# SerCharles/CN-RMA

Measured on AMD Instinct MI355X. Metric: scenes/sec fwd (40-view->192^3 voxel): dense unprojection + RMA + voxelise + FCAF3D + decode, higher is better.
Workload: dtype f32 (sparse conv f16x3: 22-bit operands, fp32 accumulate; value_f32_conv = exact fp32); 1 GPU; NS: 40 views x 256 ch x 480x640 fp32 maps (channels_last) -> grid 192x192x192, N=300, max_points=500000, FCAF3D MinkResNet34 + head, 1 HIP graph per scene, 3 in flight; M_rows=72216505, M_selected=500000, M_unique=496819

## Files before the change

### cn-rma_amd/csrc/dense.hip

```cpp
#include "common.h"


namespace {

static __device__ __forceinline__ int64_t ceil_div_dev(int64_t a, int64_t b) { return (a + b - 1) / b; }

struct DenseParams {
  int V, C, H, W, X, Y, Z;
  float vs, ox, oy, oz;
};

__device__ __forceinline__ void voxel_world(const DenseParams& p, int64_t g, float* wx, float* wy, float* wz) {
  const int z = (int)(g % p.Z);
  const int64_t t = g / p.Z;
  const int y = (int)(t % p.Y);
  const int x = (int)(t / p.Y);
  *wx = (float)x * p.vs + p.ox;
  *wy = (float)y * p.vs + p.oy;
  *wz = (float)z * p.vs + p.oz;
}

struct SlabOrder { int on, nsx, nsy, nsz, zt, st, tt, zi, nt, own, stagger, groups; };

__device__ __forceinline__ bool slab_decode(const DenseParams& p, const SlabOrder& o, int64_t gv, int* x, int* y, int* z) {
  const int64_t per = (int64_t)o.st * o.st * o.zt;
  const int64_t sv = gv / per;
  const int r = (int)(gv - sv * per);
  if (sv >= (int64_t)o.nsx * o.nsy * o.nsz) return false;
  const int sy = (int)(sv % o.nsy), sx = (int)((sv / o.nsy) % o.nsx), sz = (int)(sv / ((int64_t)o.nsy * o.nsx));
  const int tcols = o.tt * o.tt, zo_n = o.zt / o.zi;
  const int zin = r % o.zi, q = r / o.zi;
  const int in = q % tcols, q2 = q / tcols;
  const int zo = q2 % zo_n, tile = q2 / zo_n;
  const int zl = zo * o.zi + zin;
  const int tpr = o.st / o.tt;
  *x = sx * o.st + (tile / tpr) * o.tt + in / o.tt;
  *y = sy * o.st + (tile % tpr) * o.tt + in % o.tt;
  *z = sz * o.zt + zl;
  return *x < p.X && *y < p.Y && *z < p.Z;
}

__device__ __forceinline__ bool lattice_decode(const DenseParams& p, const SlabOrder& o, int64_t lb, int tid, int* x, int* y, int* z) {
  const int cb = o.st * o.st / 8;
  const int64_t sv = lb / cb;
  if (sv >= (int64_t)o.nsx * o.nsy * o.nsz) return false;
  const int w = (int)(lb - sv * cb), j = tid >> 5, q4 = o.st / 4;
  const int sy = (int)(sv % o.nsy), sx = (int)((sv / o.nsy) % o.nsx), sz = (int)(sv / ((int64_t)o.nsy * o.nsx));
  *x = sx * o.st + w / q4 + (o.st / 2) * (j >> 2);
  *y = sy * o.st + w % q4 + q4 * (j & 3);
  *z = sz * 32 + (tid & 31);
  return *x < p.X && *y < p.Y && *z < p.Z;
}

__device__ __forceinline__ bool project(const float* __restrict__ P, float wx, float wy, float wz, int H, int W,
                                        float* rx, float* ry) {
  float cam[3];
#pragma unroll
  for (int r = 0; r < 3; ++r) {
    float acc = P[r * 4 + 0] * wx;
    acc = fmaf(P[r * 4 + 1], wy, acc);
    acc = fmaf(P[r * 4 + 2], wz, acc);
    acc = fmaf(P[r * 4 + 3], 1.0f, acc);
    cam[r] = acc;
  }
  *rx = rintf(cam[0] / cam[2]);
  *ry = rintf(cam[1] / cam[2]);
  return (*rx >= 0.0f) && (*ry >= 0.0f) && (*rx < (float)W) && (*ry < (float)H) && (cam[2] > 0.0f);
}

template <int CT>
__global__ __launch_bounds__(256) void backproject_accum_kernel(DenseParams p, const float* __restrict__ feat,
                                                                const float* __restrict__ proj,
                                                                float* __restrict__ volume,
                                                                int32_t* __restrict__ count) {
  const int64_t G = (int64_t)p.X * p.Y * p.Z;
  const int64_t g = (int64_t)blockIdx.x * blockDim.x + threadIdx.x;
  if (g >= G) return;
  const int c0 = blockIdx.y * CT;
  float wx, wy, wz;
  voxel_world(p, g, &wx, &wy, &wz);
  float acc[CT];
#pragma unroll
  for (int c = 0; c < CT; ++c) acc[c] = 0.0f;
  int cnt = 0;
  const int64_t plane = (int64_t)p.H * p.W * p.C;
  for (int v = 0; v < p.V; ++v) {
    float rx, ry;
    if (!project(proj + v * 12, wx, wy, wz, p.H, p.W, &rx, &ry)) continue;
    ++cnt;
    const float* f = feat + v * plane + ((int64_t)(int)ry * p.W + (int)rx) * p.C + c0;
    if constexpr (CT % 4 == 0) {
#pragma unroll
      for (int c = 0; c < CT; c += 4) {
        float4 q = *reinterpret_cast<const float4*>(f + c);
        acc[c] += q.x; acc[c + 1] += q.y; acc[c + 2] += q.z; acc[c + 3] += q.w;
      }
    } else {
#pragma unroll
      for (int c = 0; c < CT; ++c) acc[c] += f[c];
    }
  }
  const float denom = (float)cnt;
#pragma unroll
  for (int c = 0; c < CT; ++c) {
    if (c0 + c < p.C) volume[(int64_t)(c0 + c) * G + g] = cnt > 0 ? acc[c] / denom : 0.0f;
  }
  if (blockIdx.y == 0) count[g] = cnt;
}

__device__ __forceinline__ void group_barrier(unsigned int* w, unsigned int n) {
  __syncthreads();
  if (threadIdx.x == 0) {
    const unsigned int old = __hip_atomic_fetch_add(w, 1u, __ATOMIC_RELAXED, __HIP_MEMORY_SCOPE_AGENT);
    const unsigned int goal = (old / n + 1u) * n;
    for (int spin = 0; spin < 1024; ++spin) {
      if ((int)(__hip_atomic_load(w, __ATOMIC_RELAXED, __HIP_MEMORY_SCOPE_AGENT) - goal) >= 0) break;
      __builtin_amdgcn_s_sleep(64);
    }
  }
  __syncthreads();
}

template <int LPV, int EPI>
__device__ __forceinline__ int group_src_lane(int grp, int vsel) {
  constexpr int VPG = 64 / LPV;
  if constexpr (EPI == 0 && LPV >= 4) return (grp / 4) * (4 * VPG) + vsel * 4 + (grp % 4);
  else return grp * VPG + vsel;
}

typedef float dense_f4 __attribute__((ext_vector_type(4)));

template <int ELEM> struct DenseElem { typedef float type; typedef float4 load_t; static constexpr int Q = 1; };
template <> struct DenseElem<CNRMA_ELEM_F16> { typedef uint16_t type; typedef uint4 load_t; static constexpr int Q = 2; };
template <> struct DenseElem<CNRMA_ELEM_BF16> { typedef uint16_t type; typedef uint4 load_t; static constexpr int Q = 2; };

__device__ __forceinline__ void store_run(float* o, float a, float b, float c, float d, int policy) {
  dense_f4 v = {a, b, c, d};
  if (policy == 1) __builtin_nontemporal_store(v, reinterpret_cast<dense_f4*>(o));
  else if (policy == 2) asm volatile("global_store_dwordx4 %0, %1, off sc1\n\ts_nop 1" : : "v"(o), "v"(v) : "memory");
  else *reinterpret_cast<dense_f4*>(o) = v;
}

template <int LPV, int PIPE, int EPI, int ELEM = 0>
__device__ __forceinline__ void accum_block(const DenseParams& p, const typename DenseElem<ELEM>::type* __restrict__ feat,
                                            const float* __restrict__ proj, float* __restrict__ volume,
                                            int32_t* __restrict__ count, int64_t lb, int c0, bool write_count,
                                            const SlabOrder& ord, float* __restrict__ lds_wave, int tid) {
  constexpr int VPG = 64 / LPV;
  constexpr int Q = DenseElem<ELEM>::Q, CPL = 4 * Q;
  typedef typename DenseElem<ELEM>::type feat_t;
  typedef typename DenseElem<ELEM>::load_t load_t;
  static_assert(EPI != 1 || ELEM == 0, "the LDS-transposed epilogue exists for fp32 maps only");
  const int64_t G = (int64_t)p.X * p.Y * p.Z;
  const int lane = tid & 63;
  const int64_t g = lb * 256 + tid;
  float wx = 0.f, wy = 0.f, wz = 0.f;
  bool in_grid;
  int64_t lin = -1;
  if (ord.on) {
    int x = 0, y = 0, z = 0;
    in_grid = ord.on == 2 ? lattice_decode(p, ord, lb, tid, &x, &y, &z) : slab_decode(p, ord, g, &x, &y, &z);
    if (in_grid) {
      lin = ((int64_t)x * p.Y + y) * p.Z + z;
      wx = (float)x * p.vs + p.ox; wy = (float)y * p.vs + p.oy; wz = (float)z * p.vs + p.oz;
    }
  } else {
    in_grid = g < G;
    if (in_grid) { voxel_world(p, g, &wx, &wy, &wz); lin = g; }
  }
  if (__ballot(in_grid) == 0ull) return;
  float4 acc[LPV * Q];
#pragma unroll
  for (int i = 0; i < LPV * Q; ++i) acc[i] = make_float4(0.f, 0.f, 0.f, 0.f);
  int cnt = 0;
  int sub = lane % LPV, vsel = lane / LPV;
  const int64_t plane = (int64_t)p.H * p.W * p.C;
  const feat_t* fbase = feat + c0 + CPL * sub;

  auto pixel_of = [&](int v) -> int {
    float rx, ry;
    const bool ok = in_grid && project(proj + v * 12, wx, wy, wz, p.H, p.W, &rx, &ry);
    return ok ? ((int)ry * p.W + (int)rx) : -1;
  };
  auto gather = [&](int v, int pix, load_t* q) {
    const feat_t* fv = fbase + v * plane;
#pragma unroll
    for (int grp = 0; grp < LPV; ++grp) {
      const int pq = __shfl(pix, group_src_lane<LPV, EPI>(grp, vsel), 64);
      if constexpr (ELEM == 0) q[grp] = make_float4(0.f, 0.f, 0.f, 0.f);
      else q[grp] = make_uint4(0u, 0u, 0u, 0u);
      if (pq >= 0) q[grp] = *reinterpret_cast<const load_t*>(fv + (int64_t)pq * p.C);
    }
  };
  auto add = [&](const load_t* q) {
#pragma unroll
    for (int grp = 0; grp < LPV; ++grp) {
      if constexpr (ELEM == 0) {
        acc[grp].x += q[grp].x; acc[grp].y += q[grp].y; acc[grp].z += q[grp].z; acc[grp].w += q[grp].w;
      } else {
        float4 a, b;
        elem16_x8<ELEM>(q[grp], &a, &b);
        acc[2 * grp].x += a.x; acc[2 * grp].y += a.y; acc[2 * grp].z += a.z; acc[2 * grp].w += a.w;
        acc[2 * grp + 1].x += b.x; acc[2 * grp + 1].y += b.y; acc[2 * grp + 1].z += b.z; acc[2 * grp + 1].w += b.w;
      }
    }
  };

  if constexpr (PIPE == 1) {
    int pix_n = pixel_of(0);
    for (int v = 0; v < p.V; ++v) {
      const int pix = pix_n;
      const bool any = __ballot(pix >= 0) != 0ull;
      load_t q[LPV];
      if (any) gather(v, pix, q);
      cnt += pix >= 0 ? 1 : 0;
      pix_n = (v + 1 < p.V) ? pixel_of(v + 1) : -1;
      if (any) add(q);
    }
  } else {
    load_t q0[LPV], q1[LPV];
    int pix0 = pixel_of(0);
    bool any0 = __ballot(pix0 >= 0) != 0ull;
    if (any0) gather(0, pix0, q0);
    cnt += pix0 >= 0 ? 1 : 0;
    for (int v = 0; v < p.V; ++v) {
      bool any1 = false;
      if (v + 1 < p.V) {
        const int pix1 = pixel_of(v + 1);
        any1 = __ballot(pix1 >= 0) != 0ull;
        if (any1) gather(v + 1, pix1, q1);
        cnt += pix1 >= 0 ? 1 : 0;
      }
      if (any0) add(q0);
      any0 = any1;
#pragma unroll
      for (int grp = 0; grp < LPV; ++grp) q0[grp] = q1[grp];
    }
  }

  if constexpr (ELEM != 0 && LPV >= 8) {
    int t2 = tid;
    asm volatile("" : "+v"(t2));
    sub = (t2 & 63) % LPV; vsel = (t2 & 63) / LPV;
    int x = 0, y = 0, z = 0;
    const int64_t g2 = lb * 256 + t2;
    bool in2;
    if (ord.on) in2 = ord.on == 2 ? lattice_decode(p, ord, lb, t2, &x, &y, &z) : slab_decode(p, ord, g2, &x, &y, &z);
    else { in2 = g2 < G; z = (int)(g2 % p.Z); y = (int)((g2 / p.Z) % p.Y); x = (int)(g2 / p.Z / p.Y); }
    in_grid = in2;
    lin = in2 ? ((int64_t)x * p.Y + y) * p.Z + z : -1;
  }
  if constexpr (EPI == 0 && LPV >= 4) {
    const bool vec_ok = (G & 3) == 0 && (reinterpret_cast<uintptr_t>(volume) & 15) == 0;
    const int c = c0 + CPL * sub;
#pragma unroll
    for (int r = 0; r < LPV / 4; ++r) {
      int64_t gv[4];
      float m[4][CPL];
#pragma unroll
      for (int k = 0; k < 4; ++k) {
        const int src = group_src_lane<LPV, EPI>(4 * r + k, vsel);
        const int cv = __shfl(cnt, src, 64);
        const int lo = __shfl((int)(lin & 0xffffffffLL), src, 64), hi = __shfl((int)(lin >> 32), src, 64);
        gv[k] = ((int64_t)hi << 32) | (uint32_t)lo;
        const float denom = (float)cv;
#pragma unroll
        for (int h = 0; h < Q; ++h) {
          const float4 a = acc[(4 * r + k) * Q + h];
          m[k][4 * h + 0] = cv > 0 ? a.x / denom : 0.0f; m[k][4 * h + 1] = cv > 0 ? a.y / denom : 0.0f;
          m[k][4 * h + 2] = cv > 0 ? a.z / denom : 0.0f; m[k][4 * h + 3] = cv > 0 ? a.w / denom : 0.0f;
        }
      }
      const bool whole = vec_ok && gv[0] >= 0 && (gv[0] & 3) == 0 && gv[1] == gv[0] + 1 && gv[2] == gv[0] + 2 && gv[3] == gv[0] + 3;
      if (whole) {
        float* o = volume + (int64_t)c * G + gv[0];
#pragma unroll
        for (int j = 0; j < CPL; ++j) store_run(o + j * G, m[0][j], m[1][j], m[2][j], m[3][j], ord.nt);
      } else {
#pragma unroll
        for (int k = 0; k < 4; ++k)
          if (gv[k] >= 0) {
            float* o = volume + (int64_t)c * G + gv[k];
#pragma unroll
            for (int j = 0; j < CPL; ++j) o[j * G] = m[k][j];
          }
      }
    }
  } else if constexpr (EPI != 1) {
#pragma unroll
    for (int grp = 0; grp < LPV; ++grp) {
      const int src = group_src_lane<LPV, EPI>(grp, vsel);
      const int cv = __shfl(cnt, src, 64);
      const int lo = __shfl((int)(lin & 0xffffffffLL), src, 64), hi = __shfl((int)(lin >> 32), src, 64);
      const int64_t gv = ((int64_t)hi << 32) | (uint32_t)lo;
      if (gv >= 0) {
        const float denom = (float)cv;
#pragma unroll
        for (int h = 0; h < Q; ++h) {
          const float4 a = acc[grp * Q + h];
          const int c = c0 + CPL * sub + 4 * h;
          const float m0 = cv > 0 ? a.x / denom : 0.0f, m1 = cv > 0 ? a.y / denom : 0.0f, m2 = cv > 0 ? a.z / denom : 0.0f,
                      m3 = cv > 0 ? a.w / denom : 0.0f;
          float* o = volume + (int64_t)c * G + gv;
          if (ord.nt == 1) {
            __builtin_nontemporal_store(m0, o); __builtin_nontemporal_store(m1, o + G);
            __builtin_nontemporal_store(m2, o + 2 * G); __builtin_nontemporal_store(m3, o + 3 * G);
          } else { o[0] = m0; o[G] = m1; o[2 * G] = m2; o[3 * G] = m3; }
        }
      }
    }
  } else {
    constexpr int LD = 65;
    int t2 = tid;
    asm volatile("" : "+v"(t2));
    const int lane2 = t2 & 63, sub2 = lane2 % LPV, vsel2 = lane2 / LPV;
    float* ldsw = lds_wave + 0 * (t2 & 0);
#pragma unroll
    for (int grp = 0; grp < LPV; ++grp) {
      const int cv = __shfl(cnt, grp * VPG + vsel2, 64);
      const float denom = (float)cv;
      const float4 a = acc[grp];
      float* t = ldsw + (4 * sub2) * LD + grp * VPG + vsel2;
      t[0 * LD] = cv > 0 ? a.x / denom : 0.0f;
      t[1 * LD] = cv > 0 ? a.y / denom : 0.0f;
      t[2 * LD] = cv > 0 ? a.z / denom : 0.0f;
      t[3 * LD] = cv > 0 ? a.w / denom : 0.0f;
    }
    __builtin_amdgcn_wave_barrier();
    if (in_grid) {
      float* o = volume + (int64_t)c0 * G + lin;
#pragma unroll
      for (int c = 0; c < 4 * LPV; ++c) o[(int64_t)c * G] = ldsw[c * LD + lane2];
    }
    __builtin_amdgcn_wave_barrier();
  }
  if (write_count && in_grid) count[lin] = cnt;
}

template <int LPV, int PIPE, int EPI, int LOCK>
__global__ __launch_bounds__(256, PIPE == 1 ? 4 : 3) void backproject_accum_pipe_kernel(DenseParams p, const float* feat,
                                                                     const float* __restrict__ proj,
                                                                     float* __restrict__ volume,
                                                                     int32_t* __restrict__ count, int chunk_blocks,
                                                                     int64_t n_phys, SlabOrder ord,
                                                                     unsigned int* __restrict__ bar,
                                                                     const float* const* __restrict__ feat_ref) {
  if (feat_ref != nullptr) feat = *feat_ref;
  __shared__ float lds[EPI == 1 ? 4 * (4 * LPV) * 65 : 1];
  float* lds_wave = lds + (EPI == 1 ? (threadIdx.x >> 6) * (4 * LPV) * 65 : 0);
  if constexpr (LOCK != 0) {
    const int NG = ord.groups;
    const int grp = blockIdx.x % NG, slot = blockIdx.x / NG;
    const int64_t n_chunks = n_phys / chunk_blocks;
    const int n_sweeps = (int)ceil_div_dev(p.C, 4 * LPV);
    for (int sw = 0; sw < n_sweeps; ++sw)
      for (int64_t ch = grp; ch < n_chunks; ch += NG) {
        for (int i = 0; i < ord.stagger * (int)(threadIdx.x >> 6); ++i) __builtin_amdgcn_s_sleep(1);
        int tid = threadIdx.x;
        asm volatile("" : "+v"(tid));
        accum_block<LPV, PIPE, EPI>(p, feat, proj, volume, count, ch * chunk_blocks + slot, sw * 4 * LPV, sw == 0, ord, lds_wave, tid);
        group_barrier(bar + grp * 16, (unsigned)chunk_blocks);
      }
  } else {
    int64_t lb = blockIdx.x;
    int sweep = blockIdx.y;
    if (ord.own > 0) {
      sweep = (int)(lb & 7);
      lb >>= 3;
    } else if (chunk_blocks > 0) {
      const int64_t grp = lb & 7, k = lb >> 3;
      lb = (grp + 8 * (k / chunk_blocks)) * chunk_blocks + k % chunk_blocks;
    }
    accum_block<LPV, PIPE, EPI>(p, feat, proj, volume, count, lb, sweep * (4 * LPV), sweep == 0, ord, lds_wave, (int)threadIdx.x);
  }
}

template <int LPV, int ELEM, int OCC>
__global__ __launch_bounds__(256, OCC) void backproject_accum_h16_kernel(DenseParams p, const uint16_t* feat,
                                                                         const float* __restrict__ proj,
                                                                         float* __restrict__ volume,
                                                                         int32_t* __restrict__ count, int chunk_blocks,
                                                                         SlabOrder ord,
                                                                         const uint16_t* const* __restrict__ feat_ref) {
  if (feat_ref != nullptr) feat = *feat_ref;
  int64_t lb = blockIdx.x;
  if (chunk_blocks > 0) {
    const int64_t grp = lb & 7, k = lb >> 3;
    lb = (grp + 8 * (k / chunk_blocks)) * chunk_blocks + k % chunk_blocks;
  }
  const int sweep = blockIdx.y;
  accum_block<LPV, 1, 0, ELEM>(p, feat, proj, volume, count, lb, sweep * (8 * LPV), sweep == 0, ord, nullptr, (int)threadIdx.x);
}

#ifdef CNRMA_EXPERIMENTS
#include "dense_exp.inc"
#endif

struct DenseTune {
  int variant = 1;
  int slab = 1;
  int st = 16, zt = 32, tt = 8, zi = 32;
  int chunk = -1;
  int persist = 0;
  int lpv = 0;
  int pipe = 1;
  int epi = 0;
  int nt = 0;
  int own = 0;
  int stagger = 0;
  int ldspad = 0;
  int groups = 8;
  int lattice = 0;
  int lockstep = 0;
  int zrun = 1;
};
#ifdef CNRMA_EXPERIMENTS
static DenseTune g_tune;
#define CNRMA_DENSE_TUNE g_tune
#else
static constexpr DenseTune k_dense_tune{};
#define CNRMA_DENSE_TUNE k_dense_tune
#endif

template <int LPV>
int launch_accum_coop(const DenseParams& p, const float* feat, const float* proj, float* volume, int32_t* count,
                      unsigned int* bar, hipStream_t st, const float* const* feat_ref = nullptr) {
  const DenseTune t = CNRMA_DENSE_TUNE;
  if (feat_ref != nullptr && t.variant != 1) return CNRMA_EINVAL;
  const int64_t G = (int64_t)p.X * p.Y * p.Z;
  int64_t nb = ceil_div(G, 256);
  int64_t cb = ceil_div((int64_t)p.Y * p.Z, 256);
  if (cb < 32) cb = 32;
  SlabOrder ord{0, 0, 0, 0, t.zt, t.st, t.tt, t.zi, t.nt, 0, t.stagger, t.groups == 16 ? 16 : 8};
  if (t.slab) {
    ord.on = 1;
    if (ord.zi < 1 || ord.zt % ord.zi != 0) return CNRMA_EINVAL;
    if (ord.zt < 1 || ord.tt < 1 || ord.st < ord.tt || ord.st % ord.tt != 0 || ((int64_t)ord.st * ord.st * ord.zt) % 256 != 0) return CNRMA_EINVAL;
    ord.nsx = (int)ceil_div(p.X, ord.st); ord.nsy = (int)ceil_div(p.Y, ord.st); ord.nsz = (int)ceil_div(p.Z, ord.zt);
    cb = (int64_t)ord.st * ord.st * ord.zt / 256;
    nb = (int64_t)ord.nsx * ord.nsy * ord.nsz * cb;
  } else if (t.chunk >= 0) cb = t.chunk;
  int64_t gx = nb;
  if (cb > 0 && (nb >= 16 * cb || ord.on)) gx = ceil_div(ceil_div(nb, cb), 8) * 8 * cb;
  else cb = 0;
#ifdef CNRMA_EXPERIMENTS
  if (t.variant == 0) {
    int64_t launch_x = gx;
    if (t.persist > 0 && gx > (int64_t)256 * t.persist) launch_x = (int64_t)256 * t.persist;
    dim3 grid((unsigned)launch_x, (unsigned)ceil_div(p.C, 4 * LPV));
    hipLaunchKernelGGL((backproject_accum_coop_kernel<LPV>), grid, dim3(256), 0, st, p, feat, proj, volume, count, (int)cb, gx, ord);
    CNRMA_LAUNCH_CHECK();
    return 0;
  }
  if (t.variant == 2 && p.V <= 64 && (int64_t)p.H * p.W * p.C * 4 < ((int64_t)1 << 31)) {
    const int lock = (t.lockstep && (bar != nullptr || t.lockstep == 2) && ord.on && ord.zt == 32 && ord.st % 8 == 0 && cb > 0 && cb <= 256) ? 1 : 0;
    const size_t lds = (size_t)4 * p.V * 64 * sizeof(int32_t);
    dim3 grid(lock ? (unsigned)(8 * cb) : (unsigned)gx);
    if (lock)
      hipLaunchKernelGGL((backproject_accum_hoist_kernel<LPV, 1>), grid, dim3(256), lds, st, p, feat, proj, volume, count, (int)cb,
                         gx, ord, bar, t.lockstep == 1 ? 1 : 0);
    else
      hipLaunchKernelGGL((backproject_accum_hoist_kernel<LPV, 0>), grid, dim3(256), lds, st, p, feat, proj, volume, count, (int)cb,
                         gx, ord, bar, 0);
    CNRMA_LAUNCH_CHECK();
    return 0;
  }
#endif
  const int lock = (t.lockstep == 1 && bar != nullptr && ord.on && cb > 0 && cb <= 256) ? 1 : 0;
  if (t.lattice && ord.on && ord.zt == 32 && ord.st % 8 == 0) ord.on = 2;
  const int n_sweeps = (int)ceil_div(p.C, 4 * LPV);
  if (t.own && !lock && ord.on && n_sweeps == 8 && nb * 8 < ((int64_t)1 << 31)) ord.own = 1;
  dim3 grid(lock ? (unsigned)(ord.groups * cb) : (ord.own ? (unsigned)(nb * 8) : (unsigned)gx), (lock || ord.own) ? 1u : (unsigned)n_sweeps);
#ifdef CNRMA_EXPERIMENTS
#define CNRMA_DENSE_LAUNCH(PIPE, EPI)                                                                                      \
  do {                                                                                                                     \
    if (lock)                                                                                                              \
      hipLaunchKernelGGL((backproject_accum_pipe_kernel<LPV, PIPE, EPI, 1>), grid, dim3(256), 0, st, p, feat, proj, volume, \
                         count, (int)cb, gx, ord, bar, feat_ref);                                                          \
    else                                                                                                                   \
      hipLaunchKernelGGL((backproject_accum_pipe_kernel<LPV, PIPE, EPI, 0>), grid, dim3(256), (size_t)t.ldspad * 1024, st, p,  \
                         feat, proj, volume, count, (int)cb, gx, ord, bar, feat_ref);                                     \
  } while (0)
  if (t.pipe == 2) { if (t.epi) CNRMA_DENSE_LAUNCH(2, 1); else if (t.zrun) CNRMA_DENSE_LAUNCH(2, 0); else CNRMA_DENSE_LAUNCH(2, 2); }
  else             { if (t.epi) CNRMA_DENSE_LAUNCH(1, 1); else if (t.zrun) CNRMA_DENSE_LAUNCH(1, 0); else CNRMA_DENSE_LAUNCH(1, 2); }
#undef CNRMA_DENSE_LAUNCH
#else
  (void)lock;
  hipLaunchKernelGGL((backproject_accum_pipe_kernel<LPV, 1, 0, 0>), grid, dim3(256), 0, st, p, feat, proj, volume, count, (int)cb, gx,
                     ord, bar, feat_ref);
#endif
  CNRMA_LAUNCH_CHECK();
  return 0;
}

__global__ __launch_bounds__(256) void backproject_index_kernel(DenseParams p, const float* __restrict__ proj,
                                                                int32_t* __restrict__ px, int32_t* __restrict__ py,
                                                                uint8_t* __restrict__ valid) {
  const int64_t G = (int64_t)p.X * p.Y * p.Z;
  const int64_t g = (int64_t)blockIdx.x * blockDim.x + threadIdx.x;
  if (g >= G) return;
  float wx, wy, wz, rx, ry;
  voxel_world(p, g, &wx, &wy, &wz);
  bool ok = project(proj, wx, wy, wz, p.H, p.W, &rx, &ry);
  const float lim = 2147483000.0f;
  px[g] = (rx > -lim && rx < lim) ? (int32_t)rx : INT32_MIN;
  py[g] = (ry > -lim && ry < lim) ? (int32_t)ry : INT32_MIN;
  valid[g] = ok ? 1 : 0;
}

template <int CT>
int launch_accum(const DenseParams& p, const float* feat, const float* proj, float* volume, int32_t* count,
                 hipStream_t st) {
  const int64_t G = (int64_t)p.X * p.Y * p.Z;
  dim3 grid((unsigned)ceil_div(G, 256), (unsigned)ceil_div(p.C, CT));
  hipLaunchKernelGGL((backproject_accum_kernel<CT>), grid, dim3(256), 0, st, p, feat, proj, volume, count);
  CNRMA_LAUNCH_CHECK();
  return 0;
}

}

#ifdef CNRMA_EXPERIMENTS
extern "C" int cnrma_debug_dense_tuning(const int* v, int n) {
  DenseTune t;
  int* f[] = {&t.variant, &t.slab, &t.st, &t.zt, &t.tt, &t.zi, &t.chunk, &t.persist, &t.lpv, &t.pipe, &t.epi, &t.lockstep, &t.lattice, &t.nt, &t.own, &t.stagger, &t.groups, &t.ldspad, &t.zrun};
  if (n < 0 || n > 19 || (n > 0 && v == nullptr)) return CNRMA_EINVAL;
  for (int i = 0; i < n; ++i) *f[i] = v[i];
  g_tune = t;
  return 0;
}
#endif

static int backproject_accum_any(const float* feat_nhwc, const float* const* feat_ref, const float* proj, int V, int C, int H,
                                 int W, int X, int Y, int Z, float voxel_size, float ox, float oy, float oz, float* volume,
                                 int32_t* count, void* workspace, int64_t workspace_bytes, void* stream) {
  if (V <= 0 || C <= 0 || H <= 0 || W <= 0 || X <= 0 || Y <= 0 || Z <= 0) return CNRMA_EINVAL;
  DenseParams p{V, C, H, W, X, Y, Z, voxel_size, ox, oy, oz};
  hipStream_t st = as_stream(stream);
  unsigned int* bar = (workspace != nullptr && workspace_bytes >= CNRMA_DENSE_WORKSPACE_BYTES) ? static_cast<unsigned int*>(workspace) : nullptr;
#ifdef CNRMA_EXPERIMENTS
  const int l = CNRMA_DENSE_TUNE.lpv;
  if (l == 16 && C % 64 == 0) return launch_accum_coop<16>(p, feat_nhwc, proj, volume, count, bar, st, feat_ref);
  if (l == 4 && C % 16 == 0) return launch_accum_coop<4>(p, feat_nhwc, proj, volume, count, bar, st, feat_ref);
#endif
  if (C % 32 == 0) return launch_accum_coop<8>(p, feat_nhwc, proj, volume, count, bar, st, feat_ref);
  if (C % 16 == 0) return launch_accum_coop<4>(p, feat_nhwc, proj, volume, count, bar, st, feat_ref);
  if (C % 8 == 0) return launch_accum_coop<2>(p, feat_nhwc, proj, volume, count, bar, st, feat_ref);
  if (C % 4 == 0) return launch_accum_coop<1>(p, feat_nhwc, proj, volume, count, bar, st, feat_ref);
  if (feat_ref != nullptr) return CNRMA_EINVAL;
  return launch_accum<1>(p, feat_nhwc, proj, volume, count, st);
}

extern "C" int cnrma_backproject_accum_f32(const float* feat_nhwc, const float* proj, int V, int C, int H, int W,
                                           int X, int Y, int Z, float voxel_size, float ox, float oy, float oz,
                                           float* volume, int32_t* count, void* workspace, int64_t workspace_bytes,
                                           void* stream) {
  if (feat_nhwc == nullptr) return CNRMA_EINVAL;
  return backproject_accum_any(feat_nhwc, nullptr, proj, V, C, H, W, X, Y, Z, voxel_size, ox, oy, oz, volume, count, workspace,
                               workspace_bytes, stream);
}

extern "C" int cnrma_backproject_accum_ref_f32(const float* const* feat_nhwc_ref, const float* proj, int V, int C, int H, int W,
                                               int X, int Y, int Z, float voxel_size, float ox, float oy, float oz,
                                               float* volume, int32_t* count, void* workspace, int64_t workspace_bytes,
                                               void* stream) {
  if (feat_nhwc_ref == nullptr || C % 4 != 0) return CNRMA_EINVAL;
  return backproject_accum_any(nullptr, feat_nhwc_ref, proj, V, C, H, W, X, Y, Z, voxel_size, ox, oy, oz, volume, count,
                               workspace, workspace_bytes, stream);
}

#define CNRMA_H16_LANES_C64 4

template <int LPV, int OCC>
static int launch_accum_h16(const DenseParams& p, const uint16_t* feat, const uint16_t* const* feat_ref, int elem, const float* proj,
                            float* volume, int32_t* count, hipStream_t st) {
  constexpr DenseTune t{};
  SlabOrder ord{1, (int)ceil_div(p.X, t.st), (int)ceil_div(p.Y, t.st), (int)ceil_div(p.Z, t.zt), t.zt, t.st, t.tt, t.zi, t.nt, 0, 0, 8};
  const int64_t cb = (int64_t)t.st * t.st * t.zt / 256;
  const int64_t nb = (int64_t)ord.nsx * ord.nsy * ord.nsz * cb;
  const int64_t gx = ceil_div(ceil_div(nb, cb), 8) * 8 * cb;
  dim3 grid((unsigned)gx, (unsigned)ceil_div(p.C, 8 * LPV));
  if (elem == CNRMA_ELEM_F16)
    hipLaunchKernelGGL((backproject_accum_h16_kernel<LPV, CNRMA_ELEM_F16, OCC>), grid, dim3(256), 0, st, p, feat, proj, volume, count,
                       (int)cb, ord, feat_ref);
  else
    hipLaunchKernelGGL((backproject_accum_h16_kernel<LPV, CNRMA_ELEM_BF16, OCC>), grid, dim3(256), 0, st, p, feat, proj, volume, count,
                       (int)cb, ord, feat_ref);
  CNRMA_LAUNCH_CHECK();
  return 0;
}

extern "C" int cnrma_backproject_accum_h16(const void* feat_nhwc, const void* const* feat_nhwc_ref, int elem, const float* proj,
                                           int V, int C, int H, int W, int X, int Y, int Z, float voxel_size, float ox, float oy,
                                           float oz, float* volume, int32_t* count, void* workspace, int64_t workspace_bytes,
                                           void* stream) {
  (void)workspace; (void)workspace_bytes;
  if (!elem16_known(elem) || (feat_nhwc == nullptr) == (feat_nhwc_ref == nullptr) || (reinterpret_cast<uintptr_t>(feat_nhwc) & 15) != 0)
    return CNRMA_EINVAL;
  if (V <= 0 || C <= 0 || C % 8 != 0 || H <= 0 || W <= 0 || X <= 0 || Y <= 0 || Z <= 0) return CNRMA_EINVAL;
  DenseParams p{V, C, H, W, X, Y, Z, voxel_size, ox, oy, oz};
  hipStream_t st = as_stream(stream);
  const uint16_t* f = static_cast<const uint16_t*>(feat_nhwc);
  const uint16_t* const* fr = reinterpret_cast<const uint16_t* const*>(feat_nhwc_ref);
#if defined(CNRMA_EXPERIMENTS) || CNRMA_H16_LANES_C64 == 8
  int lanes64 = CNRMA_H16_LANES_C64;
#ifdef CNRMA_EXPERIMENTS
  if (CNRMA_DENSE_TUNE.lpv == 8 || CNRMA_DENSE_TUNE.lpv == 4) lanes64 = CNRMA_DENSE_TUNE.lpv;
#endif
  if (C % 64 == 0 && lanes64 == 8) return launch_accum_h16<8, 3>(p, f, fr, elem, proj, volume, count, st);
#endif
  if (C % 32 == 0) return launch_accum_h16<4, 4>(p, f, fr, elem, proj, volume, count, st);
  if (C % 16 == 0) return launch_accum_h16<2, 4>(p, f, fr, elem, proj, volume, count, st);
  return launch_accum_h16<1, 4>(p, f, fr, elem, proj, volume, count, st);
}

template <int LPV>
__global__ __launch_bounds__(256) void backproject_backward_kernel(DenseParams p, const float* __restrict__ grad_volume,
                                                                   const int32_t* __restrict__ count,
                                                                   const float* __restrict__ proj,
                                                                   float* __restrict__ grad_feat) {
  const int64_t G = (int64_t)p.X * p.Y * p.Z;
  const int64_t t = (int64_t)blockIdx.x * blockDim.x + threadIdx.x;
  const int64_t g = t / LPV;
  const int sub = (int)(t % LPV);
  if (g >= G) return;
  const int cnt = count[g];
  if (cnt <= 0) return;
  float wx, wy, wz;
  voxel_world(p, g, &wx, &wy, &wz);
  const float denom = (float)cnt;
  const int64_t plane = (int64_t)p.H * p.W * p.C;
  for (int c = 4 * sub; c < p.C; c += 4 * LPV) {
    float gq[4];
#pragma unroll
    for (int j = 0; j < 4; ++j) gq[j] = (c + j < p.C) ? grad_volume[(int64_t)(c + j) * G + g] / denom : 0.0f;
    for (int v = 0; v < p.V; ++v) {
      float rx, ry;
      if (!project(proj + v * 12, wx, wy, wz, p.H, p.W, &rx, &ry)) continue;
      float* q = grad_feat + v * plane + ((int64_t)(int)ry * p.W + (int)rx) * p.C + c;
#pragma unroll
      for (int j = 0; j < 4; ++j)
        if (c + j < p.C) atomicAdd(q + j, gq[j]);
    }
  }
}

extern "C" int cnrma_backproject_backward_f32(const float* grad_volume, const int32_t* count, const float* proj, int V,
                                              int C, int H, int W, int X, int Y, int Z, float voxel_size, float ox,
                                              float oy, float oz, float* grad_feat_nhwc, void* stream) {
  if (V <= 0 || C <= 0 || H <= 0 || W <= 0 || X <= 0 || Y <= 0 || Z <= 0 || grad_volume == nullptr || count == nullptr ||
      grad_feat_nhwc == nullptr)
    return CNRMA_EINVAL;
  DenseParams p{V, C, H, W, X, Y, Z, voxel_size, ox, oy, oz};
  hipStream_t st = as_stream(stream);
  hipError_t e = cnrma_fill_bytes(grad_feat_nhwc, 0, (size_t)V * H * W * C * sizeof(float), st);
  if (e != hipSuccess) return -(int)e;
  const int64_t G = (int64_t)X * Y * Z;
  if (C >= 32) {
    hipLaunchKernelGGL((backproject_backward_kernel<8>), dim3((unsigned)ceil_div(G * 8, 256)), dim3(256), 0, st, p,
                       grad_volume, count, proj, grad_feat_nhwc);
  } else {
    hipLaunchKernelGGL((backproject_backward_kernel<1>), dim3((unsigned)ceil_div(G, 256)), dim3(256), 0, st, p, grad_volume,
                       count, proj, grad_feat_nhwc);
  }
  CNRMA_LAUNCH_CHECK();
  return 0;
}

extern "C" int cnrma_backproject_index_f32(const float* proj_view, int H, int W, int X, int Y, int Z, float voxel_size,
                                           float ox, float oy, float oz, int32_t* px, int32_t* py, uint8_t* valid,
                                           void* stream) {
  if (H <= 0 || W <= 0 || X <= 0 || Y <= 0 || Z <= 0) return CNRMA_EINVAL;
  DenseParams p{1, 1, H, W, X, Y, Z, voxel_size, ox, oy, oz};
  const int64_t G = (int64_t)X * Y * Z;
  hipLaunchKernelGGL(backproject_index_kernel, dim3((unsigned)ceil_div(G, 256)), dim3(256), 0, as_stream(stream), p,
                     proj_view, px, py, valid);
  CNRMA_LAUNCH_CHECK();
  return 0;
}
```

### cn-rma_amd/pipeline.py

```python
import torch

from . import _lib, rma
from . import plan as P
from . import sparse as S


DEFER_POINT_FEATURES = True
DENSE_BRANCH = False


class SceneConfig:
    def __init__(self, dims, voxel_size=0.04, origin=(0.0, 0.0, 0.0), stride=4, n_steps=300, thr=0.05,
                 max_points=500000, voxel_size_fcaf3d=0.01, ray_marching_type="neus", depth_points=None,
                 sampler="device", sample_seed=None):
        self.dims = tuple(dims)
        self.voxel_size = voxel_size
        self.origin = tuple(origin)
        self.stride = stride
        self.n_steps = n_steps
        self.thr = thr
        self.max_points = max_points
        self.voxel_size_fcaf3d = voxel_size_fcaf3d
        self.ray_marching_type = ray_marching_type
        self.depth_points = depth_points
        self.sampler = sampler
        self.sample_seed = sample_seed


def graph_node_count(graph):
    import ctypes
    import os
    try:
        hip = ctypes.CDLL(os.path.join(os.path.dirname(torch.__file__), "lib", "libamdhip64.so"))
        n = ctypes.c_size_t(0)
        hip.hipGraphGetNodes.argtypes = [ctypes.c_void_p, ctypes.c_void_p, ctypes.POINTER(ctypes.c_size_t)]
        hip.hipGraphGetNodes.restype = ctypes.c_int
        if hip.hipGraphGetNodes(ctypes.c_void_p(graph.raw_cuda_graph()), None, ctypes.byref(n)) != 0:
            return None
        return int(n.value)
    except Exception:
        return None


def weight_tensors(*modules):
    import itertools
    return [t for m in modules for t in itertools.chain(m.parameters(), m.buffers())]


def weights_tag(tensors):
    v = 0
    for t in tensors:
        v += t._version
    return (len(tensors), v, tensors[0].data_ptr() if tensors else 0)


def _offset_list(offset):
    if offset is None:
        return (0.0, 0.0, 0.0)
    return tuple(float(x) for x in torch.as_tensor(offset, dtype=torch.float32).detach().reshape(3).cpu().tolist())


class StageTimer:

    def __init__(self, enabled):
        self.enabled = enabled
        self.marks = []

    def mark(self, name):
        if self.enabled:
            e = torch.cuda.Event(enable_timing=True)
            e.record()
            self.marks.append((name, e))

    def result(self):
        if not self.enabled:
            return {}
        torch.cuda.synchronize()
        out = {}
        for (_, a), (n, b) in zip(self.marks[:-1], self.marks[1:]):
            out[n] = out.get(n, 0.0) + a.elapsed_time(b)
        return out


@torch.no_grad()
def forward_scenes(cfg, backbone, head, scenes):
    parts, infos, states = [], [], []
    for sc_ in scenes:
        feats = rma.to_nhwc(sc_["features"])
        volume, count = rma.backproject_accum(feats, sc_["projection"], cfg.dims, cfg.voxel_size, cfg.origin, cfg.stride)
        proj_inv = rma.projection_inverse(sc_["projection"], cfg.stride).to(feats.device, non_blocking=True)
        states.append(rma.aggregate_begin(feats, proj_inv, sc_["tsdf"], cfg.dims, cfg.voxel_size, cfg.origin, cfg.n_steps,
                                          cfg.thr, cfg.ray_marching_type, cfg.depth_points))
        infos.append(dict(volume=volume, count=count))
    reads = _lib.read_ints(torch.cat([st["readback"] for st in states]))
    w = len(reads) // len(scenes)
    for b, (sc_, st) in enumerate(zip(scenes, states)):
        coords, pfeats, info = rma.aggregate_finish(st, reads[b * w:(b + 1) * w], sc_.get("offset", (0.0, 0.0, 0.0)),
                                                    cfg.max_points, cfg.sampler, sc_.get("mask"))
        parts.append((coords, pfeats))
        infos[b].update(info)
    x = S.sparse_collate(parts, cfg.voxel_size_fcaf3d)
    levels = backbone(x)
    cen, box, cls, pts, scn = map(list, head(levels, fused=True))
    dets = head.get_bboxes_fused(cen, box, cls, pts, scn, len(scenes))
    outs = []
    for b, (bboxes, scores) in enumerate(dets):
        outs.append(dict(bboxes=bboxes, scores=scores, M=infos[b]["M"], M_selected=infos[b]["M_selected"],
                         M_unique=x.cs.batch_counts()[b], volume=infos[b]["volume"], count=infos[b]["count"],
                         level_rows=[len(l) for l in levels], head_rows=[len(c[0]) for c in cen]))
    return outs


@torch.no_grad()
def forward_scene(cfg, backbone, head, features_nchw, projections, tsdf, offset=(0.0, 0.0, 0.0), dense=True,
                  timing=False, mask=None, proj_inv=None, keep_half=False):
    tm = StageTimer(timing)
    tm.mark("start")
    feats = rma.to_nhwc(features_nchw, keep_dtype=keep_half)
    tm.mark("nhwc")
    out = {}
    if dense:
        volume, count = rma.backproject_accum(feats, projections, cfg.dims, cfg.voxel_size, cfg.origin, cfg.stride)
        out["volume"], out["count"] = volume, count
        tm.mark("dense")
    if proj_inv is None:
        proj_inv = rma.projection_inverse(projections, cfg.stride)
    proj_inv = proj_inv.to(feats.device, non_blocking=True)
    coords, pfeats, info = rma.aggregate_points(
        feats, proj_inv, tsdf, cfg.dims, cfg.voxel_size, cfg.origin, cfg.n_steps, cfg.thr, cfg.ray_marching_type,
        cfg.depth_points, offset=offset, max_points=cfg.max_points, sampler=cfg.sampler, mask=mask, seed=cfg.sample_seed)
    tm.mark("rma")
    x, _ = S.voxelize(coords, pfeats, cfg.voxel_size_fcaf3d)
    if P.current() is not None:
        P.current().mark("net")
    tm.mark("voxelize")
    levels = backbone(x)
    tm.mark("backbone")
    cen, box, cls, pts = map(list, head(levels))
    tm.mark("head")
    bboxes, scores = head._get_bboxes_single([c[0] for c in cen], [b[0] for b in box], [c[0] for c in cls],
                                             [p[0] for p in pts])
    tm.mark("decode")
    out.update(bboxes=bboxes, scores=scores, M=info["M"], M_selected=info["M_selected"], M_unique=len(x),
               level_rows=[len(l) for l in levels], head_rows=[len(c[0]) for c in cen], stage_ms=tm.result())
    return out


def trace_nms(plan, out, nms, state, nms_pre=0):
    from . import postprocess
    b, sc, sizes = out["bboxes"], out["scores"], list(out["sizes"])
    if nms_pre > 0 and any(k > nms_pre for k in sizes):
        starts = [sum(sizes[:l]) for l in range(len(sizes))]
        sizes = [min(k, nms_pre) for k in sizes]
        b = torch.cat([b[r0:r0 + k] for r0, k in zip(starts, sizes)])
        sc = torch.cat([sc[r0:r0 + k] for r0, k in zip(starts, sizes)])
    if b.shape[0] > postprocess.NMS_DEVICE_MAX_ROWS:
        raise _lib.CnrmaError(f"nms= needs a detection block of at most {postprocess.NMS_DEVICE_MAX_ROWS} rows, the plan's "
                              f"levels {sizes} add up to {b.shape[0]}")
    key = (b.shape[0], sc.shape[1], b.shape[1], b.device)
    if state.get("key") != key:
        state.clear()
        state.update(key=key, bufs=postprocess.nms_device_buffers(b.shape[0], sc.shape[1], b.shape[1], b.device))
    bufs = state["bufs"]
    plan.keep(*bufs.values())
    boxes, scores, labels, n = postprocess.nms_device(b, sc, valid=out["valid"], sizes=sizes, padded=True, out=bufs, **nms)
    out.update(nms_boxes=boxes, nms_scores=scores, nms_labels=labels, nms_n=n)


def check_nms_setting(nms):
    if nms is not None and not (isinstance(nms, dict) and set(nms) <= {"score_thr", "iou_thr"}):
        raise ValueError(f"nms must be None or dict(score_thr=..., iou_thr=...), got {nms!r}")
    return None if nms is None else dict(nms)


def final_detections(out):
    if "nms_n" not in out:
        raise _lib.CnrmaError("this static trace was built without nms=...: it ends at the raw detections")
    if out.get("done") is not None:
        torch.cuda.current_stream(out["bboxes"].device).wait_event(out["done"])
    host = _lib.read_ints(torch.cat((out["status"].view(-1), out["valid"].view(-1), out["counts"].view(-1),
                                     out["nms_n"].view(-1))))
    if host[0] != 0:
        raise _lib.CnrmaError(f"{host[0]} capacity / branch assumption(s) of the static plan violated: re-run eagerly")
    k = min(host[-1], out["nms_boxes"].shape[0])
    return out["nms_boxes"][:k], out["nms_scores"][:k], out["nms_labels"][:k]


def trace_net(plan, backbone, head, coords, feats, n_dev, voxel_size, device, extra_counts=(), late=None, nms=None,
              nms_state=None):
    if feats is None:
        rec_f = late["rec"].view(torch.float32)
        xr, _ = S.voxelize(coords, rec_f, voxel_size, n_dev=n_dev)
        amax = S._amax_slot(device)
        F = rma.emit_point_features(late, xr.F.view(torch.int32), xr.cs.n, xr.cs.n_dev, amax=amax)
        x = S.SparseTensor(F, xr.cs, None, amax)
    else:
        x, _ = S.voxelize(coords, feats, voxel_size, n_dev=n_dev)
    levels = backbone(x)
    cen, box, cls, pts, css = map(list, head(levels, fused=True))
    bboxes, scores, valid, sizes = head.get_bboxes_static(cen, box, cls, pts, css)
    status = plan.status(device)
    counts = torch.cat([c.view(1) for c in extra_counts] + [x.cs.n_dev.view(1)] + [l.cs.n_dev.view(1) for l in levels] +
                       [c[0].n_dev.view(1) for c in css]).to(torch.int32)
    out = dict(bboxes=bboxes, scores=scores, valid=valid, sizes=sizes, status=status, counts=counts, n_levels=len(levels),
               n_extra=len(extra_counts), levels=levels,
               head=dict(centerness=[c[0] for c in cen], bbox_pred=[b[0] for b in box], cls_score=[c[0] for c in cls],
                         points=[p[0] for p in pts], n_dev=[c[0].n_dev for c in css]))
    if nms is not None:
        trace_nms(plan, out, nms, nms_state, (head.test_cfg.nms_pre or 0) if head.test_cfg is not None else 0)
    return out


class StaticNet:

    def __init__(self, backbone, head, voxel_size, device, margin=1.2, stream=None, nms=None):
        self.backbone, self.head, self.voxel_size = backbone, head, voxel_size
        self.nms, self._nms_state = check_nms_setting(nms), {}
        self.device = torch.device(device)
        self.margin = margin
        self.stream = stream if stream is not None else torch.cuda.Stream(device=self.device)
        self.plan = self.graph = self.out = None

    def build(self, coords, feats, capture=True, cap=None):
        _lib.require_gpu()
        self._enter(coords, feats)
        with torch.cuda.stream(self.stream), torch.no_grad():
            plan = P.Plan(self.margin)
            with P.using(plan):
                x, _ = S.voxelize(coords, feats, self.voxel_size)
                levels = self.backbone(x)
                cen, box, cls, pts = map(list, self.head(levels))
                bboxes, scores = self.head._get_bboxes_single([c[0] for c in cen], [b[0] for b in box], [c[0] for c in cls],
                                                              [p[0] for p in pts])
            self.plan = plan
            M, C = feats.shape
            self.cap = int(cap or M)
            self.coords = torch.zeros((self.cap, 3), dtype=torch.float32, device=self.device)
            self.feats = torch.zeros((self.cap, C), dtype=torch.float32, device=self.device)
            self.n_dev = torch.zeros(1, dtype=torch.int32, device=self.device)
            self._load(coords, feats)
            self.out = self._trace()
            self.stream.synchronize()
            if capture:
                self.graph = torch.cuda.CUDAGraph()
                with torch.cuda.graph(self.graph, stream=self.stream):
                    self.out = self._trace()
                self.stream.synchronize()
        return dict(bboxes=bboxes, scores=scores, level_rows=[len(l) for l in levels])

    def _load(self, coords, feats):
        n = coords.shape[0]
        assert n <= self.cap
        self.coords[:n].copy_(coords, non_blocking=True)
        self.feats[:n].copy_(feats, non_blocking=True)
        self.n_dev.fill_(n)

    def _trace(self):
        self.plan.begin_static()
        with P.using(self.plan), torch.no_grad():
            out = trace_net(self.plan, self.backbone, self.head, self.coords, self.feats, self.n_dev, self.voxel_size,
                            self.device, nms=self.nms, nms_state=self._nms_state)
        self.plan.end_static()
        return out

    def _enter(self, *inputs):
        cur = torch.cuda.current_stream(self.device)
        if cur != self.stream:
            self.stream.wait_stream(cur)
            for t in inputs:
                if torch.is_tensor(t) and t.is_cuda:
                    t.record_stream(self.stream)

    def run(self, coords, feats):
        self._enter(coords, feats)
        with torch.cuda.stream(self.stream):
            self._load(coords, feats)
            if self.graph is not None:
                self.graph.replay()
            else:
                self.out = self._trace()
            self.done = torch.cuda.Event()
            self.done.record()
        self.out["done"] = self.done
        return self.out

    final_detections = staticmethod(final_detections)


class StaticScene:

    def __init__(self, cfg, backbone, head, device, margin=1.2, dense=True, stream=None, by_reference=True,
                 feature_dtype=torch.float32, nms=None):
        self.cfg, self.backbone, self.head = cfg, backbone, head
        self.nms, self._nms_state = check_nms_setting(nms), {}
        self.feature_dtype = feature_dtype
        if feature_dtype != torch.float32:
            if feature_dtype not in rma.ELEM_CODES:
                raise ValueError(f"feature_dtype must be torch.float32, torch.float16 or torch.bfloat16, got {feature_dtype}")
            if cfg.ray_marching_type != "neus":
                raise ValueError("16-bit feature maps are read by the NeuS path only: depth mode takes a float32 slot")
        self.device = torch.device(device)
        self.margin, self.dense = margin, dense
        self.by_reference = bool(by_reference)
        self.stream = stream if stream is not None else torch.cuda.Stream(device=self.device)
        self.graph = None
        self.plan = None
        self.out = None
        self._copied = None
        self.check_weights = True
        self._weights = weight_tensors(backbone, head)
        self._tag = None

    def _alloc_inputs(self, features_nchw, tsdf):
        V, C, H, W = features_nchw.shape
        dev = self.device
        if self.feature_dtype != torch.float32 and C % 8 != 0:
            raise ValueError(f"a {self.feature_dtype} slot needs C % 8 == 0 (one 16-byte load is 8 channels), got C = {C}")
        self.shape_nhwc = (V, H, W, C)
        self.nhwc = None
        self.feat_ref = torch.zeros(1, dtype=torch.int64, device=dev)
        self._pin_ref = torch.zeros(1, dtype=torch.int64, pin_memory=True)
        self._held = None
        self.proj_scaled = torch.empty((V, 3, 4), dtype=torch.float32, device=dev)
        self.proj_inv = torch.empty((V, 4, 4), dtype=torch.float32, device=dev)
        self.tsdf = torch.empty(tuple(self.cfg.dims), dtype=torch.float32, device=dev)
        self.seed_dev = torch.zeros(1, dtype=torch.int32, device=dev)
        self.offset_dev = torch.zeros(3, dtype=torch.float32, device=dev)
        self._pin_off = torch.zeros(3, dtype=torch.float32, pin_memory=True)
        cfg = self.cfg
        self.march = self.march_out = None
        if cfg.ray_marching_type == "neus":
            self.march = rma._March(None, self.proj_inv, self.tsdf, cfg.dims, cfg.voxel_size, cfg.origin, cfg.n_steps,
                                    cfg.thr, "neus", 0, shape=self.shape_nhwc, device=dev, feat_ref=self.feat_ref,
                                    feat_dtype=self.feature_dtype)
            if self.march.kept_cap() <= 0:
                raise _lib.CnrmaError("the static trace needs the single-march NeuS path (thr > 1/62)")
            self.march_out = self.march.march_buffers()
        else:
            self._nhwc_buffer()
        self._pin_proj = torch.empty((V, 3, 4), dtype=torch.float32, pin_memory=True)
        self._pin_inv = torch.empty((V, 4, 4), dtype=torch.float32, pin_memory=True)

    def _nhwc_buffer(self):
        if self.nhwc is None:
            self.nhwc = torch.empty(self.shape_nhwc, dtype=self.feature_dtype, device=self.device)
            if self.march is not None:
                self.march.feat = self.nhwc
        return self.nhwc

    def _load(self, features_nchw, projections, tsdf, proj_inv=None, offset=None, by_reference=None):
        if features_nchw is not None and self.feature_dtype != torch.float32 and features_nchw.dtype != self.feature_dtype:
            raise ValueError(f"this slot reads {self.feature_dtype} feature maps, got {features_nchw.dtype}: convert them "
                             "explicitly or use a slot of their dtype")
        if self._copied is not None:
            self._copied.synchronize()
        p = projections.detach().to("cpu", torch.float32)
        self._pin_proj.copy_(rma.scale_projection(p, self.cfg.stride))
        self._pin_inv.copy_(rma.projection_inverse(p, self.cfg.stride) if proj_inv is None
                            else proj_inv.detach().to("cpu", torch.float32))
        self.proj_scaled.copy_(self._pin_proj, non_blocking=True)
        self.proj_inv.copy_(self._pin_inv, non_blocking=True)
        self.tsdf.copy_(tsdf.reshape(self.tsdf.shape), non_blocking=True)
        if offset is None:
            self._pin_off.zero_()
        else:
            self._pin_off.copy_(torch.as_tensor(offset, dtype=torch.float32).detach().reshape(3).cpu())
        self.offset_dev.copy_(self._pin_off, non_blocking=True)
        layout_from = None
        by_reference = self.by_reference if by_reference is None else bool(by_reference)
        self._held = None
        in_place = rma.is_channels_last(features_nchw, (self.feature_dtype,))
        if in_place and self.feature_dtype != torch.float32 and features_nchw.data_ptr() % 16 != 0:
            by_reference = False
        if features_nchw is None:
            addr = self._nhwc_buffer().data_ptr()
        elif in_place and self.march is not None and by_reference:
            assert tuple(features_nchw.shape) == (self.shape_nhwc[0], self.shape_nhwc[3], self.shape_nhwc[1], self.shape_nhwc[2])
            addr = features_nchw.data_ptr()
            self._held = features_nchw
        elif in_place:
            self._nhwc_buffer().copy_(features_nchw.permute(0, 2, 3, 1), non_blocking=True)
            addr = self.nhwc.data_ptr()
        else:
            addr = self._nhwc_buffer().data_ptr()
            layout_from = features_nchw
        self._pin_ref[0] = addr
        self.feat_ref.copy_(self._pin_ref, non_blocking=True)
        self._copied = torch.cuda.Event()
        self._copied.record()
        if self.march is not None:
            self.march.march(layout_from=layout_from, into=self.march_out)
        elif layout_from is not None:
            rma.to_nhwc(layout_from, out=self.nhwc)
        self._consumed = torch.cuda.Event()
        self._consumed.record()

    def _enter(self, *inputs):
        cur = torch.cuda.current_stream(self.device)
        if cur != self.stream:
            self.stream.wait_stream(cur)
            for t in inputs:
                if torch.is_tensor(t) and t.is_cuda:
                    t.record_stream(self.stream)

    def _trace(self):
        cfg, plan = self.cfg, self.plan
        plan.begin_static()
        out = {}
        with P.using(plan), torch.no_grad():
            side = None
            if self.dense:
                main = torch.cuda.current_stream(self.device)
                if DENSE_BRANCH:
                    if getattr(self, "_side", None) is None:
                        self._side = torch.cuda.Stream(device=self.device)
                    side = self._side
                    side.wait_stream(main)
                with torch.cuda.stream(side if side is not None else main):
                    out["volume"], out["count"] = rma.backproject_accum(None, None, cfg.dims, cfg.voxel_size, cfg.origin,
                                                                        cfg.stride, proj_scaled=self.proj_scaled,
                                                                        feat_ref=self.feat_ref, shape=self.shape_nhwc,
                                                                        feat_dtype=self.feature_dtype)
            fixed = cfg.sample_seed is not None
            coords, feats, n_sel, info = rma.aggregate_points_static(
                self.nhwc, self.proj_inv, self.tsdf, cfg.dims, cfg.voxel_size, cfg.origin, cfg.n_steps, cfg.thr,
                max_points=cfg.max_points, seed=cfg.sample_seed if fixed else 0x5EED,
                seed_dev=None if fixed else self.seed_dev,
                marched=(self.march, self.march_out) if self.march is not None else None,
                mode=cfg.ray_marching_type, select_grids=cfg.depth_points or 0, feat_ref=self.feat_ref, shape=self.shape_nhwc,
                defer_feats=DEFER_POINT_FEATURES, feat_dtype=self.feature_dtype)
            moved = coords + self.offset_dev
            out.update(trace_net(plan, self.backbone, self.head, moved, feats, n_sel, cfg.voxel_size_fcaf3d, self.device,
                                 extra_counts=[info["M"], n_sel], late=info, nms=self.nms, nms_state=self._nms_state))
            if not fixed:
                self.seed_dev.add_(1)
            if side is not None:
                torch.cuda.current_stream(self.device).wait_stream(side)
        plan.end_static()
        out.update(points=(coords, feats, n_sel), points_info=info if feats is None else None)
        return out

    @staticmethod
    def point_features(out):
        coords, feats, n_sel = out["points"]
        if feats is None:
            if out.get("done") is not None:
                torch.cuda.current_stream(coords.device).wait_event(out["done"])
            feats = rma.point_features(out["points_info"])
        return feats

    def calibrate(self, features_nchw, projections, tsdf, proj_inv=None, offset=None):
        _lib.require_gpu()
        self._enter(features_nchw, tsdf)
        with torch.cuda.stream(self.stream):
            plan = P.Plan(self.margin)
            with P.using(plan):
                eager = forward_scene(self.cfg, self.backbone, self.head, features_nchw, projections, tsdf, dense=self.dense,
                                      proj_inv=proj_inv, offset=_offset_list(offset),
                                      keep_half=self.feature_dtype != torch.float32)
        self.plan = plan if self.plan is None else self.plan.merge(plan)
        return eager

    def build(self, features_nchw, projections, tsdf, capture=True, plan=None, proj_inv=None):
        _lib.require_gpu()
        eager = None
        if plan is not None:
            self.plan = P.Plan(self.margin)
            self.plan.sizes, self.plan.flags, self.plan.marks = list(plan.sizes), list(plan.flags), dict(plan.marks)
        elif self.plan is None:
            eager = self.calibrate(features_nchw, projections, tsdf, proj_inv)
        self._enter(features_nchw, tsdf)
        with torch.cuda.stream(self.stream):
            self._alloc_inputs(features_nchw, tsdf)
            self._load(features_nchw, projections, tsdf, proj_inv)
            self.out = self._trace()
            self.stream.synchronize()
            if capture:
                try:
                    self.graph, kept = torch.cuda.CUDAGraph(keep_graph=True), True
                except TypeError:
                    self.graph, kept = torch.cuda.CUDAGraph(), False
                with torch.cuda.graph(self.graph, stream=self.stream):
                    self.out = self._trace()
                self.n_nodes = graph_node_count(self.graph) if kept else None
                self.arena_fallbacks = self.plan.arena_fallbacks
                if kept:
                    self.graph.instantiate()
                self.stream.synchronize()
        self._tag = weights_tag(self._weights)
        return eager

    def run(self, features_nchw, projections, tsdf, proj_inv=None, offset=None, by_reference=None):
        if self.graph is not None and self.check_weights and weights_tag(self._weights) != self._tag:
            raise _lib.CnrmaError("the model's weights changed since this scene graph was captured (optimiser step, "
                                  "load_state_dict, .to()): the graph replays prepared weight images -- rebuild() it")
        self._enter(features_nchw, tsdf)
        with torch.cuda.stream(self.stream):
            self._load(features_nchw, projections, tsdf, proj_inv, offset, by_reference)
            consumed = self._consumed
            if self.graph is not None:
                self.graph.replay()
            else:
                self.out = self._trace()
            self.done = torch.cuda.Event()
            self.done.record()
        self.out["done"] = self.done
        self.out["inputs_consumed"] = self.done if self._held is not None else consumed
        return self.out

    def rebuild(self, features_nchw, projections, tsdf):
        if getattr(self, "outgrown", None) is not None:
            self.plan.static = False
            self.plan = self.plan.merge(self.outgrown) if len(self.plan.sizes) == len(self.outgrown.sizes) else self.outgrown
            self.outgrown, self.n_outgrown = None, 0
        fresh = P.Plan(self.margin)
        fresh.sizes, fresh.flags, fresh.marks = list(self.plan.sizes), list(self.plan.flags), dict(self.plan.marks)
        self.plan = None
        return self.build(features_nchw, projections, tsdf, capture=True, plan=fresh)

    @staticmethod
    def detections(out):
        L = len(out["sizes"])
        if out.get("done") is not None:
            torch.cuda.current_stream(out["bboxes"].device).wait_event(out["done"])
        host = _lib.read_ints(torch.cat((out["status"].view(-1), out["valid"].view(-1), out["counts"].view(-1))))
        if host[0] != 0:
            raise _lib.CnrmaError(f"{host[0]} capacity / branch assumption(s) of the static plan violated: re-run eagerly")
        valid, counts = host[1:1 + L], host[1 + L:]
        rows, r0 = [], 0
        for k, v in zip(out["sizes"], valid):
            rows.append(torch.arange(r0, r0 + v, device=out["bboxes"].device))
            r0 += k
        rows = torch.cat(rows)
        nl, ne = out["n_levels"], out.get("n_extra", 2)
        info = dict(M_unique=counts[ne], level_rows=counts[ne + 1:ne + 1 + nl], head_rows=counts[ne + 1 + nl:ne + 1 + 2 * nl])
        if ne == 2:
            info.update(M=counts[0], M_selected=counts[1])
        return out["bboxes"].index_select(0, rows), out["scores"].index_select(0, rows), info

    final_detections = staticmethod(final_detections)

    def detect(self, features_nchw, projections, tsdf, rebuild_after=4, offset=None, by_reference=None):
        out = self.run(features_nchw, projections, tsdf, offset=offset, by_reference=by_reference)
        try:
            with torch.cuda.stream(self.stream):
                b, s, info = self.detections(out)
            info["static"] = True
            return b, s, info
        except _lib.CnrmaError:
            with torch.cuda.stream(self.stream):
                grown = P.Plan(self.margin)
                with P.using(grown):
                    e = forward_scene(self.cfg, self.backbone, self.head, features_nchw, projections, tsdf, dense=self.dense,
                                      offset=_offset_list(offset), keep_half=self.feature_dtype != torch.float32)
            prev = getattr(self, "outgrown", None)
            same = prev is not None and len(prev.sizes) == len(grown.sizes) and len(prev.flags) == len(grown.flags)
            self.outgrown = prev.merge(grown) if same else grown
            self.n_outgrown = getattr(self, "n_outgrown", 0) + 1
            info = {k: e[k] for k in ("M", "M_selected", "M_unique", "level_rows", "head_rows")}
            info["static"] = False
            if rebuild_after and self.n_outgrown >= rebuild_after:
                self.rebuild(features_nchw, projections, tsdf)
                info["rebuilt"] = True
            return e["bboxes"], e["scores"], info


class StaticBatch:

    def __init__(self, cfg, backbone, head, device, n_scenes, margin=1.2, dense=True, stream=None):
        self.cfg, self.backbone, self.head = cfg, backbone, head
        self.device = torch.device(device)
        self.B, self.margin, self.dense = int(n_scenes), margin, dense
        self.stream = stream if stream is not None else torch.cuda.Stream(device=self.device)
        self.holders = [StaticScene(cfg, backbone, head, device, margin, dense, stream=self.stream) for _ in range(self.B)]
        self.graph = self.plan = self.out = None

    def build(self, scenes, plan, capture=True):
        _lib.require_gpu()
        assert len(scenes) == self.B
        self.plan = plan.scaled(self.B)
        cur = torch.cuda.current_stream(self.device)
        if cur != self.stream:
            self.stream.wait_stream(cur)
            for sc_ in scenes:
                for t_ in (sc_[0], sc_[2]):
                    if torch.is_tensor(t_) and t_.is_cuda:
                        t_.record_stream(self.stream)
        with torch.cuda.stream(self.stream):
            for h, sc_ in zip(self.holders, scenes):
                h._alloc_inputs(sc_[0], sc_[2])
            self._load(scenes)
            self.out = self._trace()
            self.stream.synchronize()
            if capture:
                self.graph = torch.cuda.CUDAGraph()
                with torch.cuda.graph(self.graph, stream=self.stream):
                    self.out = self._trace()
                self.stream.synchronize()

    def _load(self, scenes):
        for h, sc_ in zip(self.holders, scenes):
            h._load(sc_[0], sc_[1], sc_[2], None, sc_[3] if len(sc_) > 3 else None)

    def _trace(self):
        cfg, plan, B = self.cfg, self.plan, self.B
        plan.begin_static()
        out = {}
        with P.using(plan), torch.no_grad():
            vols, pts, Ms = [], [], []
            fixed = cfg.sample_seed is not None
            for b, h in enumerate(self.holders):
                if self.dense:
                    vols.append(rma.backproject_accum(None, None, cfg.dims, cfg.voxel_size, cfg.origin, cfg.stride,
                                                      proj_scaled=h.proj_scaled, feat_ref=h.feat_ref, shape=h.shape_nhwc))
                coords, feats, n_sel, info = rma.aggregate_points_static(
                    h.nhwc, h.proj_inv, h.tsdf, cfg.dims, cfg.voxel_size, cfg.origin, cfg.n_steps, cfg.thr,
                    max_points=cfg.max_points, seed=(cfg.sample_seed if fixed else 0x5EED) + 7919 * b * (0 if fixed else 1),
                    seed_dev=None if fixed else h.seed_dev, marched=(h.march, h.march_out) if h.march is not None else None,
                    mode=cfg.ray_marching_type, select_grids=cfg.depth_points or 0, feat_ref=h.feat_ref, shape=h.shape_nhwc)
                pts.append((coords + h.offset_dev, feats, n_sel))
                Ms += [info["M"].view(1), n_sel.view(1)]
                if not fixed:
                    h.seed_dev.add_(1)
            x = S.sparse_collate_static(pts, cfg.voxel_size_fcaf3d)
            levels = self.backbone(x)
            cen, box, cls, pt, css = map(list, self.head(levels, fused=True))
            bboxes, scores, valid, sizes = self.head.get_bboxes_static_multi(cen, box, cls, pt, css, B)
            status = plan.status(self.device)
            per_level = [l.cs.counts_dev()[0] for l in levels] + [c[0].counts_dev()[0] for c in css]
            counts = torch.cat(Ms + [x.cs.counts_dev()[0]] + per_level).to(torch.int32)
        plan.end_static()
        if self.dense:
            out.update(volume=[v[0] for v in vols], count=[v[1] for v in vols])
        out.update(bboxes=bboxes, scores=scores, valid=valid, sizes=sizes, status=status, counts=counts, n_levels=len(levels))
        return out

    def run(self, scenes):
        cur = torch.cuda.current_stream(self.device)
        if cur != self.stream:
            self.stream.wait_stream(cur)
            for sc_ in scenes:
                for t_ in (sc_[0], sc_[2]):
                    if torch.is_tensor(t_) and t_.is_cuda:
                        t_.record_stream(self.stream)
        with torch.cuda.stream(self.stream):
            self._load(scenes)
            if self.graph is not None:
                self.graph.replay()
            else:
                self.out = self._trace()
            self.done = torch.cuda.Event()
            self.done.record()
        self.out["done"] = self.done
        return self.out

    def detections(self, out):
        B, L = self.B, len(out["sizes"])
        if out.get("done") is not None:
            torch.cuda.current_stream(self.device).wait_event(out["done"])
        host = _lib.read_ints(torch.cat((out["status"].view(-1), out["valid"].view(-1), out["counts"].view(-1))))
        if host[0] != 0:
            raise _lib.CnrmaError(f"{host[0]} capacity / branch assumption(s) of the static plan violated: re-run eagerly")
        valid = host[1:1 + B * L]
        counts = host[1 + B * L:]
        nl = out["n_levels"]
        res = []
        for b in range(B):
            rows, r0 = [], 0
            for k, v in zip(out["sizes"], valid[b * L:(b + 1) * L]):
                rows.append(torch.arange(r0, r0 + v, device=self.device))
                r0 += k
            rows = torch.cat(rows)
            lv = counts[2 * B + B:]
            info = dict(M=counts[2 * b], M_selected=counts[2 * b + 1], M_unique=counts[2 * B + b],
                        level_rows=[lv[l * B + b] for l in range(nl)], head_rows=[lv[(nl + l) * B + b] for l in range(nl)])
            res.append((out["bboxes"][b].index_select(0, rows), out["scores"][b].index_select(0, rows), info))
        return res


def gather_padded_detections(det, valid, det_all=None, valid_all=None):
    import torch.distributed as dist
    if not (dist.is_available() and dist.is_initialized()) or dist.get_world_size() == 1:
        return det.unsqueeze(0), valid.unsqueeze(0)
    W = dist.get_world_size()
    if det_all is None:
        det_all = torch.empty((W,) + tuple(det.shape), dtype=det.dtype, device=det.device)
        valid_all = torch.empty((W,) + tuple(valid.shape), dtype=valid.dtype, device=valid.device)
    if dist.get_backend() == "nccl":
        dist.all_gather_into_tensor(det_all, det)
        dist.all_gather_into_tensor(valid_all, valid)
    else:
        d, v = det.cpu(), valid.cpu()
        ds, vs = [torch.empty_like(d) for _ in range(W)], [torch.empty_like(v) for _ in range(W)]
        dist.all_gather(ds, d)
        dist.all_gather(vs, v)
        det_all.copy_(torch.stack(ds))
        valid_all.copy_(torch.stack(vs))
    return det_all, valid_all


def gather_detections(bboxes, scores):
    import torch.distributed as dist
    if not (dist.is_available() and dist.is_initialized()) or dist.get_world_size() == 1:
        return [(bboxes, scores)]
    W = dist.get_world_size()
    k = torch.tensor([bboxes.shape[0]], dtype=torch.int64, device=bboxes.device)
    ks = [torch.zeros_like(k) for _ in range(W)]
    dist.all_gather(ks, k)
    kmax = int(max(int(x.item()) for x in ks))
    nb, nc = bboxes.shape[1], scores.shape[1]
    block = torch.zeros((kmax, nb + nc), dtype=torch.float32, device=bboxes.device)
    block[:bboxes.shape[0], :nb] = bboxes
    block[:bboxes.shape[0], nb:] = scores
    blocks = [torch.empty_like(block) for _ in range(W)]
    dist.all_gather(blocks, block)
    return [(b[:int(n.item()), :nb], b[:int(n.item()), nb:]) for b, n in zip(blocks, ks)]
```

### cn-rma_amd/rma.py

```python
import math

import numpy as np
import torch

from . import _lib
from . import plan as P
from ._lib import call, ptr, stream


SIGMOID_TABLE = True
MARCH_SKIP = "auto"
MARCH_SKIP_MIN_RAYS = 4_000_000


def _f32(t):
    return t.contiguous().to(torch.float32)


def step_length(dims, voxel_size, n_steps):
    X, Y, Z = dims
    return math.sqrt(X ** 2 + Y ** 2 + Z ** 2) * voxel_size / n_steps


def scale_projection(projection, stride):
    p = projection.clone()
    p[..., :2, :] = p[..., :2, :] / stride
    return p


ELEM_CODES = {torch.float16: 1, torch.bfloat16: 2}


def _h16_readable(nhwc):
    return nhwc.dtype in ELEM_CODES and nhwc.shape[-1] % 8 == 0 and nhwc.data_ptr() % 16 == 0 and nhwc.is_contiguous()


def to_nhwc(features, out=None, keep_dtype=False):
    _lib.require_gpu()
    dt = features.dtype if keep_dtype and features.dtype in ELEM_CODES else torch.float32
    if out is None and is_channels_last(features, (dt,)):
        return features.permute(0, 2, 3, 1)
    features = features.contiguous() if dt != torch.float32 else _f32(features)
    V, C, H, W = features.shape
    if out is None:
        out = torch.empty((V, H, W, C), dtype=dt, device=features.device)
    assert out.shape == (V, H, W, C) and out.is_contiguous() and out.dtype == dt
    call("cnrma_nchw_to_nhwc_f32" if dt == torch.float32 else "cnrma_nchw_to_nhwc_b16", ptr(features), ptr(out), V, C, H, W, stream())
    return out


def is_channels_last(features, dtypes=(torch.float32,)):
    return (torch.is_tensor(features) and features.dim() == 4 and features.dtype in dtypes and features.is_cuda
            and features.permute(0, 2, 3, 1).is_contiguous())


def backproject_accum(features_nhwc, projections, dims, voxel_size, origin, stride, proj_scaled=None, feat_ref=None, shape=None,
                      feat_dtype=torch.float32):
    _lib.require_gpu()
    X, Y, Z = dims
    if feat_ref is not None:
        V, H, W, C = shape
        dev = feat_ref.device
    else:
        V, H, W, C = features_nhwc.shape
        dev = features_nhwc.device
    proj = proj_scaled if proj_scaled is not None else _f32(scale_projection(projections.to(torch.float32), stride)).to(dev)
    volume = torch.empty((C, X, Y, Z), dtype=torch.float32, device=dev)
    count = torch.empty((X, Y, Z), dtype=torch.int32, device=dev)
    st = stream()
    ws = _dense_workspace(dev, st)
    tail = (ptr(proj), V, C, H, W, X, Y, Z, float(voxel_size), float(origin[0]), float(origin[1]), float(origin[2]), ptr(volume),
            ptr(count), ptr(ws), ws.numel() * 4, st)
    if feat_ref is not None:
        if feat_dtype in ELEM_CODES:
            call("cnrma_backproject_accum_h16", None, ptr(feat_ref), ELEM_CODES[feat_dtype], *tail)
        else:
            call("cnrma_backproject_accum_ref_f32", ptr(feat_ref), *tail)
    elif _h16_readable(features_nhwc):
        call("cnrma_backproject_accum_h16", ptr(features_nhwc), None, ELEM_CODES[features_nhwc.dtype], *tail)
    else:
        if features_nhwc.dtype in ELEM_CODES:
            features_nhwc = _f32(features_nhwc)
        call("cnrma_backproject_accum_f32", ptr(features_nhwc), *tail)
    return volume, count


_DENSE_WS = {}
_DENSE_KEYS = ("variant", "slab", "st", "zt", "tt", "zi", "chunk", "persist", "lpv", "pipe", "epi", "lockstep", "lattice", "nt", "own", "stagger", "groups", "ldspad", "zrun")


def _dense_workspace(dev, st):
    key = (dev.index if dev.index is not None else torch.cuda.current_device(), st)
    ws = _DENSE_WS.get(key)
    if ws is None:
        if len(_DENSE_WS) >= 64:
            _DENSE_WS.pop(next(iter(_DENSE_WS)))
        ws = torch.zeros(256, dtype=torch.int32, device=dev)
        _DENSE_WS[key] = ws
    return ws


def dense_tuning(**kw):
    import ctypes
    if not kw:
        if _lib.experiments_active():
            call("cnrma_debug_dense_tuning", None, 0)
            _lib.experiments(False, "dense")
        return
    _lib.experiments(True, "dense")
    base = dict(variant=1, slab=1, st=16, zt=32, tt=8, zi=32, chunk=-1, persist=0, lpv=0, pipe=1, epi=0, lockstep=0, lattice=0, nt=0, own=0, stagger=0, groups=8, ldspad=0, zrun=1)
    base.update(DENSE_DEFAULTS)
    unknown = set(kw) - set(base)
    assert not unknown, unknown
    base.update(kw)
    arr = (ctypes.c_int * len(_DENSE_KEYS))(*[int(base[k]) for k in _DENSE_KEYS])
    call("cnrma_debug_dense_tuning", arr, len(_DENSE_KEYS))


DENSE_DEFAULTS = {}


class BackprojectAccum(torch.autograd.Function):

    @staticmethod
    def forward(ctx, features_nchw, projections, dims, voxel_size, origin, stride):
        nhwc = to_nhwc(features_nchw.detach())
        volume, count = backproject_accum(nhwc, projections, dims, voxel_size, origin, stride)
        ctx.args = (projections, tuple(dims), float(voxel_size), tuple(float(o) for o in origin), stride, nhwc.shape)
        ctx.count = count
        ctx.mark_non_differentiable(count)
        return volume, count

    @staticmethod
    def backward(ctx, grad_volume, _grad_count):
        projections, dims, vs, origin, stride, (V, H, W, C) = ctx.args
        dev = grad_volume.device
        proj = _f32(scale_projection(projections.to(torch.float32), stride)).to(dev)
        g = torch.empty((V, H, W, C), dtype=torch.float32, device=dev)
        call("cnrma_backproject_backward_f32", ptr(grad_volume.contiguous().float()), ptr(ctx.count), ptr(proj), V, C, H, W,
             dims[0], dims[1], dims[2], vs, origin[0], origin[1], origin[2], ptr(g), stream())
        return g.permute(0, 3, 1, 2).contiguous(), None, None, None, None, None


def backproject_index(projection_scaled, hw, dims, voxel_size, origin, device):
    _lib.require_gpu()
    H, W = hw
    X, Y, Z = dims
    G = X * Y * Z
    proj = _f32(projection_scaled).to(device)
    px = torch.empty(G, dtype=torch.int32, device=device)
    py = torch.empty(G, dtype=torch.int32, device=device)
    valid = torch.empty(G, dtype=torch.uint8, device=device)
    call("cnrma_backproject_index_f32", ptr(proj), H, W, X, Y, Z, float(voxel_size), float(origin[0]),
         float(origin[1]), float(origin[2]), ptr(px), ptr(py), ptr(valid), stream())
    return px, py, valid


def projection_inverse(projections, stride):
    p = scale_projection(projections.detach().to("cpu", torch.float32), stride)
    last = torch.tensor([[[0.0, 0.0, 0.0, 1.0]]]).expand(p.shape[0], 1, 4)
    return torch.inverse(torch.cat((p, last), dim=1))


def ray_params(proj_inv, H, W):
    _lib.require_gpu()
    V = proj_inv.shape[0]
    o = torch.empty((V, 3), dtype=torch.float32, device=proj_inv.device)
    d = torch.empty((V, 3, H * W), dtype=torch.float32, device=proj_inv.device)
    call("cnrma_ray_params_f32", ptr(_f32(proj_inv)), V, H, W, ptr(o), ptr(d), stream())
    return o, d


class _March:

    def __init__(self, features_nhwc, proj_inv, tsdf, dims, voxel_size, origin, n_steps, thr, mode, select_grids, shape=None,
                 device=None, feat_ref=None, feat_dtype=None):
        thr_ = float(thr) if thr is not None else 0.0
        if features_nhwc is not None:
            feat_dtype = features_nhwc.dtype
            if feat_dtype in ELEM_CODES and not (mode == "neus" and thr_ > 1.0 / 62.0 and _h16_readable(features_nhwc)):
                features_nhwc, feat_dtype = _f32(features_nhwc), torch.float32
        self.feat_dtype = feat_dtype if feat_dtype is not None else torch.float32
        self.elem = ELEM_CODES.get(self.feat_dtype, 0)
        self.feat = features_nhwc
        self.feat_ref = feat_ref
        self.V, self.H, self.W, self.C = features_nhwc.shape if features_nhwc is not None else shape
        self.dev = features_nhwc.device if features_nhwc is not None else torch.device(device)
        self.pinv = _f32(proj_inv).to(self.dev)
        self.tsdf = _f32(tsdf).to(self.dev)
        self.X, self.Y, self.Z = dims
        assert self.tsdf.numel() == self.X * self.Y * self.Z
        self.vs = float(voxel_size)
        self.org = [float(x) for x in origin]
        self.N = int(n_steps)
        self.t_one = float(step_length(dims, voxel_size, n_steps))
        self.thr = thr_
        self.mode = mode
        self.k = int(select_grids or 0)
        self.R = self.V * self.H * self.W

    def count(self):
        cnt = torch.empty(self.R, dtype=torch.int32, device=self.dev)
        wsum = torch.empty(self.R, dtype=torch.float64, device=self.dev)
        head = (ptr(self.pinv), ptr(self.tsdf), self.V, self.H, self.W, self.X, self.Y, self.Z, self.vs, *self.org,
                self.N, self.t_one)
        if self.mode == "neus":
            call("cnrma_rma_neus_count_f32", *head, self.thr, ptr(cnt), ptr(wsum), stream())
        else:
            call("cnrma_rma_depth_count_f32", *head, self.k, ptr(cnt), ptr(wsum), stream())
        return cnt, wsum

    def kept_cap(self):
        if self.mode != "neus" or not (self.thr > 1.0 / 62.0):
            return 0
        return int(1.0 / self.thr) + 2

    def march(self, layout_from=None, into=None):
        cap = self.kept_cap()
        if into is not None:
            cnt, wsum, kept, overflow, tab = into
        else:
            cnt = torch.empty(self.R, dtype=torch.int32, device=self.dev)
            wsum = torch.empty(self.R, dtype=torch.float64, device=self.dev)
            kept = torch.empty((self.R, cap, 2), dtype=torch.int32, device=self.dev)
            overflow = torch.empty(4, dtype=torch.int32, device=self.dev)
            tab = torch.empty_like(self.tsdf) if SIGMOID_TABLE else None
        overflow_all, overflow = overflow, overflow[:1]
        self._overflow = overflow
        skip = None
        if tab is not None:
            if (self.R >= MARCH_SKIP_MIN_RAYS) if MARCH_SKIP == "auto" else bool(MARCH_SKIP):
                if getattr(self, "_skip", None) is None:
                    self._skip = torch.empty(_lib.load().cnrma_rma_skip_table_bytes(self.X, self.Y, self.Z), dtype=torch.uint8,
                                             device=self.dev)
                skip = self._skip
            call("cnrma_rma_march_tables_f32", ptr(self.tsdf), self.X, self.Y, self.Z, ptr(tab), ptr(skip), stream())
        tail = (ptr(self.pinv), ptr(self.tsdf), ptr(tab), self.V, self.H, self.W, self.X, self.Y, self.Z, self.vs, *self.org,
                self.N, self.t_one, self.thr, ptr(cnt), ptr(wsum), ptr(kept), cap, ptr(overflow_all), ptr(skip), stream())
        if layout_from is not None and self.elem:
            src = layout_from.contiguous()
            assert (tuple(src.shape) == (self.V, self.C, self.H, self.W) and src.dtype == self.feat_dtype and self.feat is not None
                    and self.feat.is_contiguous() and self.feat.dtype == self.feat_dtype)
            call("cnrma_nchw_to_nhwc_b16", ptr(src), ptr(self.feat), self.V, self.C, self.H, self.W, stream())
            call("cnrma_rma_neus_march_f32", *tail)
        elif layout_from is not None:
            src = _f32(layout_from)
            assert tuple(src.shape) == (self.V, self.C, self.H, self.W) and self.feat is not None and self.feat.is_contiguous()
            call("cnrma_nchw_to_nhwc_march_f32", ptr(src), ptr(self.feat), self.C, *tail)
        else:
            call("cnrma_rma_neus_march_f32", *tail)
        return cnt, wsum, kept, overflow

    def march_buffers(self):
        cap = self.kept_cap()
        return (torch.empty(self.R, dtype=torch.int32, device=self.dev), torch.empty(self.R, dtype=torch.float64, device=self.dev),
                torch.empty((self.R, cap, 2), dtype=torch.int32, device=self.dev),
                torch.empty(4, dtype=torch.int32, device=self.dev), torch.empty_like(self.tsdf) if SIGMOID_TABLE else None)

    def _emit_rows_head(self):
        by_ref = self.feat_ref is not None
        if self.elem:
            return ("cnrma_rma_neus_emit_rows_h16", ptr(self.pinv), None if by_ref else ptr(self.feat),
                    ptr(self.feat_ref) if by_ref else None, self.elem)
        return ("cnrma_rma_neus_emit_rows_ref_f32" if by_ref else "cnrma_rma_neus_emit_rows_f32", ptr(self.pinv),
                ptr(self.feat_ref) if by_ref else ptr(self.feat))

    def emit_rows(self, row_offset, n_out, kept, sel_index, w_div, add, out_xyz, xyz_stride, out_w, w_stride, out_feat,
                  feat_stride, out_sample=None, n_out_dev=None):
        rec = torch.empty((int(n_out), 4), dtype=torch.int32, device=self.dev)
        call(*self._emit_rows_head(), self.V, self.C, self.H, self.W, self.N,
             self.t_one, ptr(row_offset), int(n_out), ptr(n_out_dev), ptr(kept), kept.shape[1], ptr(sel_index),
             sel_index.numel() if sel_index is not None else 0, ptr(rec), ptr(w_div), float(add[0]),
             float(add[1]), float(add[2]), out_xyz, xyz_stride, out_w, w_stride, out_feat, feat_stride, ptr(out_sample),
             stream())

    def emit_records(self, rec, n_out, n_out_dev, w_div, add, out_xyz, xyz_stride, out_w, w_stride, out_feat, feat_stride,
                     out_sample=None):
        call(*self._emit_rows_head(), self.V, self.C, self.H, self.W, self.N,
             self.t_one, None, int(n_out), ptr(n_out_dev), None, 0, None, 0, ptr(rec), ptr(w_div), float(add[0]),
             float(add[1]), float(add[2]), out_xyz, xyz_stride, out_w, w_stride, out_feat, feat_stride, ptr(out_sample),
             stream())

    def emit(self, row_offset, sel_index, w_div, add, out_xyz, xyz_stride, out_w, w_stride, out_feat, feat_stride,
             out_sample=None, sel_cap=0, out_cap=0):
        feat = _f32(self.feat) if self.elem else self.feat
        head = (ptr(self.pinv), ptr(self.tsdf), ptr(feat), self.V, self.C, self.H, self.W, self.X, self.Y, self.Z,
                self.vs, *self.org, self.N, self.t_one)
        tail = (ptr(row_offset), ptr(sel_index), ptr(w_div), float(add[0]), float(add[1]), float(add[2]),
                out_xyz, xyz_stride, out_w, w_stride, out_feat, feat_stride)
        if self.mode == "neus":
            call("cnrma_rma_neus_emit_f32", *head, self.thr, *tail, ptr(out_sample), stream())
        else:
            call("cnrma_rma_depth_emit_f32", *head, self.k, *tail, int(sel_cap), int(out_cap), stream())


def exclusive_scan(count):
    n = count.numel()
    out = torch.empty(n + 1, dtype=torch.int32, device=count.device)
    ws = torch.empty(_lib.load().cnrma_scan_workspace_bytes(n), dtype=torch.uint8, device=count.device)
    call("cnrma_exclusive_scan_i32", ptr(count), ptr(out), n, ptr(ws), stream())
    return out


def mask_to_index(mask_u8):
    n = mask_u8.numel()
    sel = torch.empty(n, dtype=torch.int32, device=mask_u8.device)
    n_sel = torch.empty(1, dtype=torch.int32, device=mask_u8.device)
    ws = torch.empty(_lib.load().cnrma_scan_workspace_bytes(n), dtype=torch.uint8, device=mask_u8.device)
    call("cnrma_mask_to_index", ptr(mask_u8), ptr(sel), ptr(n_sel), n, ptr(ws), stream())
    return sel, n_sel


_SAMPLE_CALLS = [0]


def sample_mask_device(m_dev, M, n_keep, seed=None, seed_dev=None):
    if seed is None:
        _SAMPLE_CALLS[0] += 1
        seed = (0x9E3779B9 * _SAMPLE_CALLS[0] + int(torch.initial_seed())) & 0xFFFFFFFF
    mask = torch.empty(M, dtype=torch.uint8, device=m_dev.device)
    ws = torch.empty(_lib.load().cnrma_sample_workspace_bytes(), dtype=torch.uint8, device=m_dev.device)
    call("cnrma_sample_mask", m_dev.data_ptr(), M, int(n_keep), int(seed), ptr(seed_dev), ptr(mask), ptr(ws), stream())
    return mask


def select_records(row_offset, kept, m_dev, M, n_keep, rec_cap, seed=None, seed_dev=None):
    if seed is None:
        _SAMPLE_CALLS[0] += 1
        seed = (0x9E3779B9 * _SAMPLE_CALLS[0] + int(torch.initial_seed())) & 0xFFFFFFFF
    dev = m_dev.device
    R = row_offset.numel() - 1
    lib = _lib.load()
    rec = torch.empty((int(rec_cap), 4), dtype=torch.int32, device=dev)
    n_sel = torch.empty(1, dtype=torch.int32, device=dev)
    ws = torch.empty(lib.cnrma_sample_workspace_bytes(), dtype=torch.uint8, device=dev)
    cnt = torch.empty(R, dtype=torch.int32, device=dev)
    off = torch.empty(R + 1, dtype=torch.int32, device=dev)
    sws = torch.empty(lib.cnrma_scan_workspace_bytes(R), dtype=torch.uint8, device=dev)
    call("cnrma_rma_select_records", ptr(row_offset), R, ptr(kept), kept.shape[1], m_dev.data_ptr(), int(M), int(n_keep),
         int(seed), ptr(seed_dev), ptr(ws), ptr(cnt), ptr(off), ptr(sws), int(rec_cap), ptr(rec), ptr(n_sel), stream())
    return rec, n_sel


def _drop_single_sample_views(cnt, wsum, V):
    call("cnrma_rma_drop_single_sample_views", ptr(cnt), ptr(wsum), int(V), cnt.numel() // int(V), stream())


def rma_view_rows(features_nhwc, proj_inv, tsdf, dims, voxel_size, origin, n_steps=300, thr=0.05, mode="neus",
                  select_grids=0, with_samples=False, single_march=None):
    _lib.require_gpu()
    m = _March(features_nhwc, proj_inv, tsdf, dims, voxel_size, origin, n_steps, thr, mode, select_grids)
    if single_march is None:
        single_march = m.kept_cap() > 0
    if single_march:
        cnt, wsum, kept, overflow = m.march()
    else:
        cnt, wsum = m.count()
    off = exclusive_scan(cnt)
    M = int(off[-1].item())
    per_view = cnt.view(m.V, -1).sum(dim=1)
    Wd = 4 + m.C
    rows = torch.empty((M, Wd), dtype=torch.float32, device=m.dev)
    samples = torch.empty((M, 2), dtype=torch.int32, device=m.dev) if with_samples else None
    if M > 0:
        base = rows.data_ptr()
        if single_march:
            assert int(overflow.item()) == 0
            m.emit_rows(off, M, kept, None, None, (0.0, 0.0, 0.0), base, Wd, base + 12, Wd, base + 16, Wd, samples)
        else:
            m.emit(off, None, None, (0.0, 0.0, 0.0), base, Wd, base + 12, Wd, base + 16, Wd, samples)
    return (rows, per_view, samples) if with_samples else (rows, per_view)


def aggregate_points(features_nhwc, proj_inv, tsdf, dims, voxel_size, origin, n_steps=300, thr=0.05, mode="neus",
                     select_grids=0, offset=(0.0, 0.0, 0.0), max_points=None, sampler="numpy", mask=None,
                     reference_quirks=True, seed=None):
    st = aggregate_begin(features_nhwc, proj_inv, tsdf, dims, voxel_size, origin, n_steps, thr, mode, select_grids,
                         reference_quirks)
    return aggregate_finish(st, _lib.read_ints(st["readback"]), offset, max_points, sampler, mask, seed)


def aggregate_begin(features_nhwc, proj_inv, tsdf, dims, voxel_size, origin, n_steps=300, thr=0.05, mode="neus",
                    select_grids=0, reference_quirks=True):
    _lib.require_gpu()
    m = _March(features_nhwc, proj_inv, tsdf, dims, voxel_size, origin, n_steps, thr, mode, select_grids)
    single_march = m.kept_cap() > 0
    kept = overflow = None
    if single_march:
        cnt, wsum, kept, overflow = m.march()
    else:
        cnt, wsum = m.count()
    if reference_quirks:
        _drop_single_sample_views(cnt, wsum, m.V)
    off = exclusive_scan(cnt)
    ws = torch.empty(_lib.load().cnrma_scan_workspace_bytes(m.R), dtype=torch.uint8, device=m.dev)
    wtot = torch.empty(1, dtype=torch.float64, device=m.dev)
    mean_w = torch.empty(1, dtype=torch.float32, device=m.dev)
    call("cnrma_sum_f64", ptr(wsum), ptr(wtot), m.R, ptr(ws), stream())
    m_total = off[m.R:]
    call("cnrma_rma_mean_weight", ptr(wtot), m_total.data_ptr(), ptr(mean_w), stream())
    readback = torch.cat((m_total, overflow)) if single_march else m_total
    return dict(m=m, single_march=single_march, cnt=cnt, off=off, kept=kept, mean_w=mean_w, m_total=m_total,
                readback=readback)


def aggregate_finish(st, readback, offset=(0.0, 0.0, 0.0), max_points=None, sampler="numpy", mask=None, seed=None):
    m, single_march, off, kept, mean_w, m_total, cnt = (st[k] for k in ("m", "single_march", "off", "kept", "mean_w",
                                                                         "m_total", "cnt"))
    M = int(readback[0])
    if single_march and readback[1]:
        raise _lib.CnrmaError("kept-sample record overflow: a ray kept more than 1/thr samples")
    if M == 0:
        raise TypeError("no valid points in any view (ray_marching.py:300)")
    if P.current() is not None:
        P.current().record(M)
    sel = None
    Ms = M
    if mask is not None or (max_points is not None and M > max_points):
        Ms = None
        if mask is None:
            Ms = int(max_points)
            if sampler == "numpy":
                mask = np.zeros(M, dtype=bool)
                mask[np.random.choice(M, max_points, replace=False)] = True
            elif sampler == "device":
                mask = sample_mask_device(m_total, M, max_points, seed=seed)
            else:
                raise ValueError(f"unknown sampler {sampler!r}")
        if isinstance(mask, np.ndarray):
            if Ms is None:
                Ms = int(mask.sum())
            mask = torch.from_numpy(mask.astype(np.uint8))
        mask = mask.to(device=m.dev, dtype=torch.uint8).contiguous()
        assert mask.numel() == M, "mask length must equal the number of aggregated rows"
        sel, n_sel = mask_to_index(mask)
        if Ms is None:
            Ms = int(n_sel.item())
    coords = torch.empty((Ms, 3), dtype=torch.float32, device=m.dev)
    feats = torch.empty((Ms, m.C), dtype=torch.float32, device=m.dev)
    if single_march:
        m.emit_rows(off, Ms, kept, sel, mean_w, offset, coords.data_ptr(), 3, None, 0, feats.data_ptr(), m.C)
    else:
        m.emit(off, sel, mean_w, offset, coords.data_ptr(), 3, None, 0, feats.data_ptr(), m.C)
    info = dict(M=M, M_selected=Ms, mean_w=mean_w, row_offset=off, count=cnt, kept=kept, sel=sel, march=m)
    return coords, feats, info


def aggregate_points_static(features_nhwc, proj_inv, tsdf, dims, voxel_size, origin, n_steps=300, thr=0.05,
                            offset=(0.0, 0.0, 0.0), max_points=None, seed=0, seed_dev=None, reference_quirks=True,
                            marched=None, mode="neus", select_grids=0, feat_ref=None, shape=None, defer_feats=False,
                            feat_dtype=None):
    plan = P.current()
    assert plan is not None and plan.static
    depth = mode == "depth"
    kept = overflow = None
    if marched is not None:
        m, (cnt, wsum, kept, overflow) = marched[0], marched[1][:4]
    elif depth:
        m = _March(features_nhwc, proj_inv, tsdf, dims, voxel_size, origin, n_steps, 0.0, "depth", select_grids)
        cnt, wsum = m.count()
    else:
        m = _March(features_nhwc, proj_inv, tsdf, dims, voxel_size, origin, n_steps, thr, "neus", 0, shape=shape,
                   device=proj_inv.device, feat_ref=feat_ref, feat_dtype=feat_dtype)
        if m.kept_cap() <= 0:
            raise _lib.CnrmaError("the static trace needs the single-march NeuS path (thr > 1/62)")
        cnt, wsum, kept, overflow = m.march()
    if reference_quirks:
        _drop_single_sample_views(cnt, wsum, m.V)
    off = exclusive_scan(cnt)
    ws = torch.empty(_lib.load().cnrma_scan_workspace_bytes(m.R), dtype=torch.uint8, device=m.dev)
    wtot = torch.empty(1, dtype=torch.float64, device=m.dev)
    mean_w = torch.empty(1, dtype=torch.float32, device=m.dev)
    call("cnrma_sum_f64", ptr(wsum), ptr(wtot), m.R, ptr(ws), stream())
    m_total = off[m.R:]
    call("cnrma_rma_mean_weight", ptr(wtot), m_total.data_ptr(), ptr(mean_w), stream())
    rows_per_ray = max(1, 2 * m.k) if depth else kept.shape[1]
    M_cap = plan.next_cap(bound=m.R * rows_per_ray, n_dev=m_total, lo=1)
    if overflow is not None:
        plan.watch(overflow, 0, 0)
    n_keep = int(max_points) if max_points is not None else M_cap
    cap = min(M_cap, n_keep)
    defer_feats = bool(defer_feats) and not depth
    coords = torch.empty((cap, 3), dtype=torch.float32, device=m.dev)
    feats = None if defer_feats else torch.empty((cap, m.C), dtype=torch.float32, device=m.dev)
    sel = rec = None
    if depth:
        mask = sample_mask_device(m_total, M_cap, n_keep, seed=seed, seed_dev=seed_dev)
        sel, n_sel = mask_to_index(mask)
        m.emit(off, sel, mean_w, offset, coords.data_ptr(), 3, None, 0, feats.data_ptr(), m.C, sel_cap=M_cap, out_cap=cap)
    else:
        rec, n_sel = select_records(off, kept, m_total, M_cap, n_keep, cap, seed=seed, seed_dev=seed_dev)
        m.emit_records(rec, cap, n_sel, mean_w, offset, coords.data_ptr(), 3, None, 0,
                       feats.data_ptr() if feats is not None else None, m.C)
    info = dict(M=m_total, M_selected=n_sel, mean_w=mean_w, row_offset=off, count=cnt, kept=kept, sel=sel, march=m, rec=rec)
    return coords, feats, n_sel, info


def emit_point_features(info, rec, n_rows, n_dev, out=None, amax=None):
    m = info["march"]
    if out is None:
        out = torch.empty((int(n_rows), m.C), dtype=torch.float32, device=m.dev)
    by_ref = m.feat_ref is not None
    head = (None if by_ref else ptr(m.feat), ptr(m.feat_ref) if by_ref else None)
    tail = (m.C, ptr(rec), int(n_rows), ptr(n_dev), ptr(info["mean_w"]), ptr(out), out.shape[1], ptr(amax), stream())
    if m.elem:
        call("cnrma_rma_emit_features_h16", *head, m.elem, *tail)
    else:
        call("cnrma_rma_emit_features_f32", *head, *tail)
    return out


def point_features(info):
    rec = info["rec"]
    return emit_point_features(info, rec, rec.shape[0], info["M_selected"])


def aggregate_points_backward(info, grad_feats):
    m, kept = info["march"], info["kept"]
    if kept is None:
        raise NotImplementedError("the backward needs the kept-sample records of the single-march forward (NeuS, thr > 1/62)")
    g = grad_feats.contiguous().float()
    out = torch.empty((m.V, m.H, m.W, m.C), dtype=torch.float32, device=m.dev)
    call("cnrma_rma_neus_rows_backward_f32", ptr(g), g.shape[1], m.V, m.C, m.H, m.W, ptr(info["row_offset"]), ptr(kept),
         kept.shape[1], ptr(info["sel"]), ptr(info["mean_w"]), ptr(out), stream())
    return out


class AggregatePoints(torch.autograd.Function):

    @staticmethod
    def forward(ctx, features_nchw, proj_inv, tsdf, dims, voxel_size, origin, n_steps, thr, offset, max_points, sampler, mask):
        nhwc = to_nhwc(features_nchw.detach())
        coords, feats, info = aggregate_points(nhwc, proj_inv, tsdf, dims, voxel_size, origin, n_steps, thr, "neus", 0,
                                               offset, max_points, sampler, mask)
        ctx.info = info
        ctx.mark_non_differentiable(coords)
        return coords, feats

    @staticmethod
    def backward(ctx, _grad_coords, grad_feats):
        g = aggregate_points_backward(ctx.info, grad_feats)
        return (g.permute(0, 3, 1, 2).contiguous(),) + (None,) * 11


def aggregate_rows(features_nhwc, proj_inv, tsdf, dims, voxel_size, origin, n_steps=300, thr=0.05, mode="neus",
                   select_grids=0, reference_quirks=True):
    coords, feats, info = aggregate_points(features_nhwc, proj_inv, tsdf, dims, voxel_size, origin, n_steps, thr, mode,
                                           select_grids, reference_quirks=reference_quirks)
    return torch.cat((coords, feats), dim=1), info


def select_rows(points, offset, mask=None):
    _lib.require_gpu()
    points = _f32(points)
    M, Wd = points.shape
    C = Wd - 3
    sel = None
    Ms = M
    if mask is not None:
        if isinstance(mask, np.ndarray):
            mask = torch.from_numpy(mask.astype(np.uint8))
        mask = mask.to(device=points.device, dtype=torch.uint8).contiguous()
        sel, _ = mask_to_index(mask)
        Ms = int(mask.sum().item())
    coords = torch.empty((Ms, 3), dtype=torch.float32, device=points.device)
    feats = torch.empty((Ms, C), dtype=torch.float32, device=points.device)
    call("cnrma_select_rows_f32", ptr(points), M, C, ptr(sel), float(offset[0]), float(offset[1]), float(offset[2]),
         ptr(coords), ptr(feats), stream())
    return coords, feats
```

### include/cnrma.h

```cpp
#ifndef CNRMA_H
#define CNRMA_H

#include <stddef.h>
#include <stdint.h>

#ifdef __cplusplus
extern "C" {
#endif

#define CNRMA_EINVAL (-22)
#define CNRMA_ABI_VERSION 7

int cnrma_abi_version(void);

int cnrma_fill_bytes_u8(void* dst, int byte, size_t n_bytes, void* stream);

int cnrma_range_violations_i32(const int32_t* values, const int32_t* lo, const int32_t* hi, int n, int32_t* out, void* stream);

int cnrma_nchw_to_nhwc_f32(const float* feat_nchw, float* feat_nhwc, int V, int C, int H, int W, void* stream);

#define CNRMA_DENSE_WORKSPACE_BYTES 1024
int cnrma_backproject_accum_f32(const float* feat_nhwc, const float* proj, int V, int C, int H, int W,
                                int X, int Y, int Z, float voxel_size, float ox, float oy, float oz,
                                float* volume, int32_t* count, void* workspace, int64_t workspace_bytes, void* stream);

int cnrma_backproject_accum_ref_f32(const float* const* feat_nhwc_ref, const float* proj, int V, int C, int H, int W,
                                    int X, int Y, int Z, float voxel_size, float ox, float oy, float oz,
                                    float* volume, int32_t* count, void* workspace, int64_t workspace_bytes, void* stream);

#define CNRMA_ELEM_F16 1
#define CNRMA_ELEM_BF16 2
int cnrma_backproject_accum_h16(const void* feat_nhwc, const void* const* feat_nhwc_ref, int elem, const float* proj, int V,
                                int C, int H, int W, int X, int Y, int Z, float voxel_size, float ox, float oy, float oz,
                                float* volume, int32_t* count, void* workspace, int64_t workspace_bytes, void* stream);
int cnrma_nchw_to_nhwc_b16(const void* feat_nchw, void* feat_nhwc, int V, int C, int H, int W, void* stream);

#ifdef CNRMA_EXPERIMENTS
int cnrma_debug_dense_tuning(const int* values, int n);
#endif

int cnrma_backproject_backward_f32(const float* grad_volume, const int32_t* count, const float* proj, int V, int C, int H,
                                   int W, int X, int Y, int Z, float voxel_size, float ox, float oy, float oz,
                                   float* grad_feat_nhwc, void* stream);

int cnrma_backproject_index_f32(const float* proj_view, int H, int W, int X, int Y, int Z, float voxel_size,
                                float ox, float oy, float oz, int32_t* px, int32_t* py, uint8_t* valid,
                                void* stream);

int cnrma_ray_params_f32(const float* proj_inv, int V, int H, int W, float* o, float* d, void* stream);

int cnrma_rma_neus_count_f32(const float* proj_inv, const float* tsdf, int V, int H, int W, int X, int Y, int Z,
                             float voxel_size, float ox, float oy, float oz, int n_steps, float t_one, float thr,
                             int32_t* count, double* wsum, void* stream);

int cnrma_rma_neus_emit_f32(const float* proj_inv, const float* tsdf, const float* feat_nhwc, int V, int C, int H,
                            int W, int X, int Y, int Z, float voxel_size, float ox, float oy, float oz, int n_steps,
                            float t_one, float thr, const int32_t* row_offset, const int32_t* sel_index,
                            const float* w_div, float addx, float addy, float addz,
                            float* out_xyz, int xyz_stride, float* out_w, int w_stride, float* out_feat,
                            int feat_stride, int32_t* out_sample, void* stream);

int cnrma_rma_sigmoid_table_f32(const float* tsdf, int64_t n, float* table, void* stream);
size_t cnrma_rma_skip_table_bytes(int X, int Y, int Z);
int cnrma_rma_march_tables_f32(const float* tsdf, int X, int Y, int Z, float* table, void* skip_table, void* stream);
#ifdef CNRMA_EXPERIMENTS
int cnrma_debug_div_by_voxel_size_f32(const float* a, int64_t n, float voxel_size, float* q_fast, float* q_ref, void* stream);
#endif
int cnrma_rma_neus_march_f32(const float* proj_inv, const float* tsdf, const float* sig_table, int V, int H, int W, int X,
                             int Y, int Z, float voxel_size, float ox, float oy, float oz, int n_steps, float t_one,
                             float thr, int32_t* count, double* wsum, void* kept, int cap, int32_t* overflow,
                             const void* skip_table, void* stream);

int cnrma_nchw_to_nhwc_march_f32(const float* feat_nchw, float* feat_nhwc, int C, const float* proj_inv, const float* tsdf,
                                 const float* sig_table, int V, int H, int W, int X, int Y, int Z, float voxel_size, float ox,
                                 float oy, float oz, int n_steps, float t_one, float thr, int32_t* count, double* wsum,
                                 void* kept, int cap, int32_t* overflow, const void* skip_table, void* stream);

int cnrma_rma_neus_rows_backward_f32(const float* grad_out_feat, int grad_stride, int V, int C, int H, int W,
                                     const int32_t* row_offset, const void* kept, int cap, const int32_t* sel_index,
                                     const float* w_div, float* grad_feat_nhwc, void* stream);
int cnrma_rma_neus_emit_rows_f32(const float* proj_inv, const float* feat_nhwc, int V, int C, int H, int W,
                                 int n_steps, float t_one, const int32_t* row_offset, int64_t n_out,
                                 const int32_t* n_out_dev, const void* kept, int cap, const int32_t* sel_index,
                                 int64_t sel_cap, void* records, const float* w_div, float addx, float addy, float addz,
                                 float* out_xyz, int xyz_stride, float* out_w, int w_stride, float* out_feat,
                                 int feat_stride, int32_t* out_sample, void* stream);
int cnrma_rma_neus_emit_rows_ref_f32(const float* proj_inv, const float* const* feat_nhwc_ref, int V, int C, int H, int W,
                                 int n_steps, float t_one, const int32_t* row_offset, int64_t n_out,
                                 const int32_t* n_out_dev, const void* kept, int cap, const int32_t* sel_index,
                                 int64_t sel_cap, void* records, const float* w_div, float addx, float addy, float addz,
                                 float* out_xyz, int xyz_stride, float* out_w, int w_stride, float* out_feat,
                                 int feat_stride, int32_t* out_sample, void* stream);
int cnrma_rma_neus_emit_rows_h16(const float* proj_inv, const void* feat_nhwc, const void* const* feat_nhwc_ref, int elem,
                                 int V, int C, int H, int W,
                                 int n_steps, float t_one, const int32_t* row_offset, int64_t n_out,
                                 const int32_t* n_out_dev, const void* kept, int cap, const int32_t* sel_index,
                                 int64_t sel_cap, void* records, const float* w_div, float addx, float addy, float addz,
                                 float* out_xyz, int xyz_stride, float* out_w, int w_stride, float* out_feat,
                                 int feat_stride, int32_t* out_sample, void* stream);

size_t cnrma_sample_workspace_bytes(void);
int cnrma_sample_mask(const int32_t* m_dev, int64_t m_cap, int n_keep, uint32_t seed, const uint32_t* seed_dev,
                      uint8_t* mask, void* workspace, void* stream);
int cnrma_rma_select_records(const int32_t* row_offset, int64_t R, const void* kept, int cap, const int32_t* m_dev,
                             int64_t m_cap, int n_keep, uint32_t seed, const uint32_t* seed_dev, void* sample_ws,
                             int32_t* ray_counts, int32_t* ray_offsets, void* scan_ws, int64_t rec_cap, void* records,
                             int32_t* n_sel, void* stream);
int cnrma_topk_mask_f32(const float* scores, const int32_t* n_dev, int64_t n_cap, int k, uint8_t* mask,
                        void* workspace, void* stream);
int cnrma_topk_indices_f32(const float* scores, const int32_t* n_dev, int64_t n_cap, int k, int64_t* out_idx,
                           void* workspace, void* stream);

int cnrma_rma_depth_count_f32(const float* proj_inv, const float* tsdf, int V, int H, int W, int X, int Y, int Z,
                              float voxel_size, float ox, float oy, float oz, int n_steps, float t_one,
                              int select_grids, int32_t* count, double* wsum, void* stream);

int cnrma_rma_depth_emit_f32(const float* proj_inv, const float* tsdf, const float* feat_nhwc, int V, int C, int H,
                             int W, int X, int Y, int Z, float voxel_size, float ox, float oy, float oz,
                             int n_steps, float t_one, int select_grids, const int32_t* row_offset,
                             const int32_t* sel_index, const float* w_div, float addx, float addy, float addz,
                             float* out_xyz, int xyz_stride, float* out_w, int w_stride, float* out_feat,
                             int feat_stride, int64_t sel_cap, int64_t out_cap, void* stream);

int cnrma_rma_drop_single_sample_views(int32_t* count, double* wsum, int V, int64_t rays_per_view, void* stream);

int cnrma_rma_mean_weight(const double* wsum_total, const int32_t* m_total, float* mean_w, void* stream);

size_t cnrma_scan_workspace_bytes(int64_t n);
int cnrma_exclusive_scan_i32(const int32_t* in, int32_t* out, int64_t n, void* workspace, void* stream);
int cnrma_sum_f64(const double* in, double* out, int64_t n, void* workspace, void* stream);
int cnrma_mask_to_index(const uint8_t* mask, int32_t* sel_index, int32_t* n_sel, int64_t n, void* workspace,
                        void* stream);

int cnrma_select_rows_f32(const float* points, int64_t M, int C, const int32_t* sel_index, float addx, float addy,
                          float addz, float* coords, float* feats, void* stream);

size_t cnrma_voxelize_workspace_bytes(int64_t M);
int cnrma_voxelize_f32(const float* coords, const float* feats, int64_t M, const int32_t* m_dev, int C,
                       float voxel_size, int batch_id, int row_order, uint64_t* hash_keys, int32_t* hash_vals,
                       int64_t hash_cap, int32_t* out_coords, float* out_feats, int32_t* out_src, int64_t out_cap,
                       int32_t* n_out, void* workspace, void* stream);


int cnrma_sparse_build_map(const int32_t* coords, int64_t n_cap, const int32_t* n_dev, uint64_t* hash_keys,
                           int32_t* hash_vals, int64_t hash_cap, int precleared ,
                           void* stream);

int cnrma_sparse_stride_coords(const int32_t* in_coords, int64_t n_cap, const int32_t* n_dev, int new_stride,
                               uint64_t* hash_keys, int32_t* hash_vals, int64_t hash_cap, int32_t* out_coords,
                               int64_t out_cap, int32_t* n_out, void* workspace, void* stream);
int cnrma_sparse_stride_coords_sorted(const int32_t* in_coords, int64_t n_cap, const int32_t* n_dev, int new_stride,
                                      int32_t* out_coords, int64_t out_cap, int32_t* n_out, void* workspace, void* stream);

int cnrma_sparse_kernel_map(const int32_t* out_coords, int64_t no_cap, const int32_t* no_dev,
                            const uint64_t* in_hash_keys, const int32_t* in_hash_vals, int64_t hash_cap,
                            const int32_t* offsets, int K, int32_t* nbr, void* stream);

int cnrma_sparse_kernel_map_symmetric(const int32_t* coords, int64_t n_cap, const int32_t* n_dev,
                                      const uint64_t* hash_keys, const int32_t* hash_vals, int64_t hash_cap,
                                      const int32_t* offsets, int K, int32_t* nbr, int precleared ,
                                      void* stream);
int cnrma_sparse_kernel_map_strided(const int32_t* in_coords, int64_t n_cap, const int32_t* n_dev, int in_stride,
                                    int kernel_size, const uint64_t* out_hash_keys, const int32_t* out_hash_vals,
                                    int64_t hash_cap, int32_t* nbr, int64_t no_cap, int precleared, void* stream);
int cnrma_sparse_kernel_map_children(const int32_t* parent_nbr, int64_t np_cap, const int32_t* np_dev, int32_t* nbr,
                                     void* stream);

size_t cnrma_sparse_conv_workspace_bytes(int64_t no_cap, int Cout, int K);
int cnrma_sparse_conv_f32(const float* in_feats, int Cin, const int32_t* nbr, int K, const float* weight, int Cout,
                          const float* scale, const float* shift, const float* residual, int act,
                          float* out_feats, int64_t no_cap, const int32_t* no_dev, void* workspace,
                          size_t workspace_bytes, void* stream);

int cnrma_sparse_conv_plan(int64_t no_cap, int Cin, int Cout, int K, int mode, int slices, size_t workspace_bytes, int* out6);
#ifdef CNRMA_EXPERIMENTS
int cnrma_debug_conv_tuning(const int* values, int n);
#endif

size_t cnrma_sparse_conv_weight_bytes(int K, int Cin, int Cout);
int cnrma_sparse_conv_prepare_weights(const float* weight, int K, int Cin, int Cout, void* weight_split, void* stream);
int cnrma_sparse_split_features(const float* feats, int64_t n_cap, const int32_t* n_dev, int C, void* out_split,
                                void* stream);
int cnrma_sparse_conv_bf16x6(const float* in_feats, const void* in_split, int64_t in_zero_row, int Cin,
                             const int32_t* nbr, int K, const void* weight_split, int Cout, const float* scale,
                             const float* shift, const float* residual, int act, float* out_feats, void* out_split,
                             int64_t no_cap, const int32_t* no_dev, void* workspace, size_t workspace_bytes,
                             void* stream);
int cnrma_sparse_convtr_gen_bf16x6(const int32_t* in_coords, const float* in_feats, const void* in_split, int64_t n_cap,
                                   const int32_t* n_dev, int Cin, int half_stride, const void* weight_split, int Cout,
                                   const float* scale, const float* shift, int act, int32_t* out_coords,
                                   float* out_feats, void* out_split, void* stream);

size_t cnrma_sparse_conv_pairs_workspace_bytes(int64_t no_cap, int K, int Cout, int64_t pair_cap);
int cnrma_sparse_conv_pairs_f16x3(const float* in_feats, const float* in_amax, int Cin, const int32_t* nbr, int K,
                                  const void* weight_split, int Cout, const float* scale, const float* shift,
                                  const float* residual, int act, float* out_feats, float* out_amax, int64_t no_cap,
                                  const int32_t* no_dev, int64_t pair_cap, void* workspace, size_t workspace_bytes,
                                  void* stream);
int cnrma_sparse_conv_pairs_f32(const float* in_feats, int Cin, const int32_t* nbr, int K, const float* weight, int Cout,
                                const float* scale, const float* shift, const float* residual, int act, float* out_feats,
                                int64_t no_cap, const int32_t* no_dev, int64_t pair_cap, void* workspace, size_t workspace_bytes,
                                void* stream);

size_t cnrma_amax_bytes(void);
int cnrma_absmax_f32(const float* in, int64_t n_cap, const int32_t* n_dev, int C, float* out_amax, void* stream);
int cnrma_rma_emit_features_f32(const float* feat_nhwc, const float* const* feat_nhwc_ref, int C, const void* records,
                                int64_t n_cap, const int32_t* n_dev, const float* w_div, float* out_feat, int feat_stride,
                                float* out_amax, void* stream);
int cnrma_rma_emit_features_h16(const void* feat_nhwc, const void* const* feat_nhwc_ref, int elem, int C, const void* records,
                                int64_t n_cap, const int32_t* n_dev, const float* w_div, float* out_feat, int feat_stride,
                                float* out_amax, void* stream);
size_t cnrma_sparse_conv_f16_weight_bytes(int K, int Cin, int Cout);
int cnrma_sparse_conv_prepare_weights_f16(const float* weight, int K, int Cin, int Cout, void* weight_split,
                                          void* stream);
int cnrma_sparse_conv_f16x3(const float* in_feats, const float* in_amax, int Cin, const int32_t* nbr, int K,
                            const void* weight_split, int Cout, const float* scale, const float* shift,
                            const float* residual, int act, float* out_feats, float* out_amax, int64_t no_cap,
                            const int32_t* no_dev, void* workspace, size_t workspace_bytes, void* stream);
size_t cnrma_sparse_tile_union_bytes(int64_t no_cap);
int cnrma_sparse_tile_union_build(const int32_t* nbr, int64_t no_cap, const int32_t* no_dev, int K, void* tile_union, void* stream);
int cnrma_sparse_conv_prepare_weights_f16_frag(const float* weight, int K, int Cin, int Cout, void* weight_frag, void* stream);
int cnrma_sparse_conv_go_f16x3(const float* in_feats, const float* in_amax, int Cin, const void* tile_union,
                               const void* weight_frag, int Cout, const float* scale, const float* shift,
                               const float* residual, int act, float* out_feats, float* out_amax, int64_t no_cap,
                               const int32_t* no_dev, void* workspace, size_t workspace_bytes, void* tile_counters,
                               void* stream);
int cnrma_sparse_conv_go_plan(int64_t no_cap, int Cin, int Cout, size_t workspace_bytes, int has_residual, int* out8);
size_t cnrma_sparse_conv_f32_frag_weight_bytes(int K, int Cin, int Cout);
int cnrma_sparse_conv_prepare_weights_f32_frag(const float* weight, int K, int Cin, int Cout, void* weight_frag, void* stream);
int cnrma_sparse_conv_go_f32(const float* in_feats, int Cin, const void* tile_union, const void* weight_frag, int Cout,
                             const float* scale, const float* shift, const float* residual, int act, float* out_feats,
                             int64_t no_cap, const int32_t* no_dev, void* workspace, size_t workspace_bytes, void* stream);
int cnrma_sparse_convtr_gen_f16x3(const int32_t* in_coords, const float* in_feats, const float* in_amax, int64_t n_cap,
                                  const int32_t* n_dev, int Cin, int half_stride, const void* weight_split, int Cout,
                                  const float* scale, const float* shift, int act, int32_t* out_coords,
                                  float* out_feats, float* out_amax, void* stream);

size_t cnrma_sparse_conv_bf16_weight_bytes(int K, int Cin, int Cout);
int cnrma_sparse_conv_prepare_weights_bf16(const float* weight, int K, int Cin, int Cout, void* weight_bf16, void* stream);
int cnrma_sparse_conv_prepare_weights_bf16_t(const float* weight, int K, int Cin, int Cout, int flip, void* weight_bf16,
                                             void* stream);
int cnrma_sparse_conv_bf16(const float* in_feats, int Cin, const int32_t* nbr, int K, const void* weight_bf16, int Cout,
                           const float* scale, const float* shift, const float* residual, int act, float* out_feats,
                           int64_t no_cap, const int32_t* no_dev, void* workspace, size_t workspace_bytes, void* stream);

int cnrma_sparse_kernel_map_transpose(const int32_t* nbr, int64_t no_cap, const int32_t* no_dev, int K, int64_t n_in,
                                      int32_t* nbr_t, void* stream);
int cnrma_sparse_conv_wgrad_chunks(int64_t no_cap, int rows_per_chunk);
int cnrma_sparse_conv_wgrad_f32(const float* in_feats, int Cin, const int32_t* nbr, int K, const float* grad_out, int Cout,
                                int64_t no_cap, const int32_t* no_dev, int rows_per_chunk, float* slabs, void* stream);
int cnrma_sparse_conv_wgrad_bf16(const float* in_feats, int Cin, const int32_t* nbr, int K, const float* grad_out, int Cout,
                                 int64_t no_cap, const int32_t* no_dev, int rows_per_chunk, float* slabs, void* stream);

int cnrma_sparse_conv_wgrad_go_bf16(const float* in_feats, int Cin, const void* tile_union, const float* grad_out, int Cout,
                                    int64_t no_cap, const int32_t* no_dev, int parts, float* slabs, void* stream);

size_t cnrma_sparse_conv_bf16_frag_weight_bytes(int K, int Cin, int Cout);
int cnrma_sparse_conv_prepare_weights_bf16_frag(const float* weight, int K, int Cin, int Cout, int transpose, int flip,
                                                void* weight_frag, void* stream);
int cnrma_sparse_conv_prepare_weights_bf16_frag_pair(const float* weight, int K, int Cin, int Cout, int flip,
                                                     void* frag_forward, void* frag_transposed, void* stream);
int cnrma_sparse_conv_go_bf16(const float* in_feats, int Cin, const void* tile_union, const void* weight_frag, int Cout,
                              float* out_feats, int64_t no_cap, const int32_t* no_dev, void* workspace, size_t workspace_bytes,
                              void* stream);

int cnrma_sparse_convtr_gen_f32(const int32_t* in_coords, const float* in_feats, int64_t n_cap, const int32_t* n_dev,
                                int Cin, int half_stride, const float* weight, int Cout, const float* scale,
                                const float* shift, int act, int32_t* out_coords, float* out_feats, void* stream);

int cnrma_sparse_maxpool_f32(const float* in_feats, int C, const int32_t* nbr, int K, float* out_feats,
                             int64_t no_cap, const int32_t* no_dev, void* stream);

size_t cnrma_instnorm_workspace_bytes(int C);
int cnrma_sparse_instnorm_f32(const float* in_feats, int64_t n_cap, const int32_t* n_dev, const int32_t* row0_dev, int C,
                              const float* weight, const float* bias, float eps, int relu, float* out_feats,
                              double* stats_ws, void* stream);
int cnrma_sparse_instnorm_maxpool_f32(const float* in_feats, int C, const double* stats, const float* weight,
                                      const float* bias, float eps, int relu, const int32_t* nbr, int K, float* out_feats,
                                      int64_t no_cap, const int32_t* no_dev, float* out_amax, void* stream);

int cnrma_bn_train_forward_f32(const float* x, int64_t n, int C, const float* weight, const float* bias, float eps,
                               const float* residual, int relu, float momentum, float* running_mean, float* running_var,
                               int64_t* num_batches_tracked, float* out, double* stats_ws, void* stream);
int cnrma_bn_train_backward_f32(const float* grad_out, const float* x, const float* y, int act, int64_t n, int C, const double* stats,
                                const float* weight, float eps, float* grad_in, float* grad_residual, float* grad_weight,
                                float* grad_bias, double* ws, void* stream);
int cnrma_bn_backward_f32(const float* grad_out, const float* x, int64_t n, int C, const double* stats, const float* weight,
                          float eps, float* grad_in, float* grad_weight, float* grad_bias, double* ws, void* stream);

size_t cnrma_union_workspace_bytes(int64_t nb);
int cnrma_sparse_union_add_f32(const int32_t* a_coords, const float* a_feats, int64_t na_cap, const int32_t* na_dev,
                               const int32_t* b_coords, const float* b_feats, int64_t nb_cap, const int32_t* nb_dev,
                               int C, uint64_t* a_hash_keys, int32_t* a_hash_vals, int64_t hash_cap,
                               int32_t* out_coords, float* out_feats, int64_t out_cap, int32_t* n_out, void* workspace,
                               void* stream);

int cnrma_sparse_interp_f32(const int32_t* q_coords, int64_t n_cap, const int32_t* n_dev, const float* score,
                            const uint64_t* s_hash_keys, const int32_t* s_hash_vals, int64_t hash_cap,
                            int score_stride, float* out, void* stream);

int cnrma_sparse_prune_f32(const int32_t* in_coords, const float* in_feats, int64_t n_cap, const int32_t* n_dev,
                           int C, const int32_t* sel_index, int32_t* out_coords, float* out_feats, void* stream);

int cnrma_rowmax_f32(const float* in, int64_t n_cap, const int32_t* n_dev, int C, float* out, void* stream);

int cnrma_fcaf3d_decode_f32(const float* points_xyz, const float* reg, int R, int64_t n, int yaw_mode,
                            float* boxes, void* stream);
int cnrma_fcaf3d_head_post_f32(const float* y, int ldy, const int32_t* coords, int64_t n, int R, int n_cls,
                               const float* scale, float voxel_size, float* centerness, float* bbox_pred, float* cls,
                               float* max_cls, float* points, void* stream);
int cnrma_fcaf3d_max_score_f32(const float* cls, const float* centerness, int64_t n, int n_cls, float* max_score,
                               void* stream);
int cnrma_fcaf3d_select_decode_f32(const int64_t* ids, int64_t k, const float* cls, const float* centerness,
                                   const float* reg, const float* points_xyz, int n_cls, int R, int yaw_mode,
                                   float* scores, float* boxes, void* stream);
int cnrma_fcaf3d_scores_f32(const float* cls, const float* centerness, int64_t n, int n_cls, float* scores,
                            float* max_score, void* stream);

int cnrma_nms_mask_f32(const float* boxes_sorted, int n, float iou_thr, int rotated, uint64_t* mask, void* stream);
int cnrma_box_iou_f32(const float* a, int na, const float* b, int nb, int rotated, int mode3d, float* iou, void* stream);

size_t cnrma_nms_classes_workspace_bytes(int n_cap, int n_cls);
int cnrma_nms_classes_f32(const float* boxes, int box_cols, const float* scores, int n_cap, int n_cls, const int32_t* sizes,
                          int n_segments, const int32_t* valid, float score_thr, float iou_thr, void* workspace,
                          size_t workspace_bytes, float* out_boxes, float* out_scores, int64_t* out_labels, int out_cap,
                          int32_t* n_out, void* stream);

#ifdef __cplusplus
}
#endif
#endif
```

Measured before the change: 62.95 scenes/s.

## Record per-wave visible-view masks on first channel sweep and skip empty views later

The dense backprojection now runs the first channel sweep as its own launch, which writes a per-wave bitmask of views that had any valid pixel into a new workspace region. The remaining sweeps read the mask and iterate only over set bits, so they skip projection and gather for views no voxel in the wave sees. Slab decoding also gets a power-of-two shift/mask fast path and 32-bit voxel index math, and gathers issue their shuffles before the loads. In exchange there is an extra kernel launch and a larger workspace allocation plumbed through Python, and the split only engages when there are enough sweeps and a workspace is passed.

```diff
diff --git a/cn-rma_amd/csrc/dense.hip b/cn-rma_amd/csrc/dense.hip
--- a/cn-rma_amd/csrc/dense.hip
+++ b/cn-rma_amd/csrc/dense.hip
@@ -11,16 +11,27 @@
 };
 
 __device__ __forceinline__ void voxel_world(const DenseParams& p, int64_t g, float* wx, float* wy, float* wz) {
-  const int z = (int)(g % p.Z);
-  const int64_t t = g / p.Z;
-  const int y = (int)(t % p.Y);
-  const int x = (int)(t / p.Y);
+  int x, y, z;
+  if (((uint64_t)g >> 32) == 0) {
+    const unsigned g32 = (unsigned)g, t = g32 / (unsigned)p.Z;
+    z = (int)(g32 - t * (unsigned)p.Z);
+    x = (int)(t / (unsigned)p.Y);
+    y = (int)(t - (unsigned)x * (unsigned)p.Y);
+  } else {
+    z = (int)(g % p.Z);
+    const int64_t t = g / p.Z;
+    y = (int)(t % p.Y);
+    x = (int)(t / p.Y);
+  }
   *wx = (float)x * p.vs + p.ox;
   *wy = (float)y * p.vs + p.oy;
   *wz = (float)z * p.vs + p.oz;
 }
 
-struct SlabOrder { int on, nsx, nsy, nsz, zt, st, tt, zi, nt, own, stagger, groups; };
+struct SlabOrder {
+  int on, nsx, nsy, nsz, zt, st, tt, zi, nt, own, stagger, groups;
+  int p2, lcb, lzi, ltt, lzo, ltpr;
+};
 
 __device__ __forceinline__ bool slab_decode(const DenseParams& p, const SlabOrder& o, int64_t gv, int* x, int* y, int* z) {
   const int64_t per = (int64_t)o.st * o.st * o.zt;
@@ -40,6 +51,33 @@
   return *x < p.X && *y < p.Y && *z < p.Z;
 }
 
+__device__ __forceinline__ bool block_decode(const DenseParams& p, const SlabOrder& o, int64_t lb, int tid, int* x, int* y, int* z) {
+  if (!o.p2) return slab_decode(p, o, lb * 256 + tid, x, y, z);
+  const unsigned b = (unsigned)lb;
+  const unsigned sv = b >> o.lcb;
+  if (sv >= (unsigned)(o.nsx * o.nsy * o.nsz)) return false;
+  const unsigned r = ((b & ((1u << o.lcb) - 1u)) << 8) | (unsigned)tid;
+  const unsigned t = sv / (unsigned)o.nsy, sy = sv - t * (unsigned)o.nsy;
+  const unsigned sz = t / (unsigned)o.nsx, sx = t - sz * (unsigned)o.nsx;
+  const unsigned zin = r & (unsigned)(o.zi - 1), q = r >> o.lzi;
+  const unsigned in = q & ((1u << (2 * o.ltt)) - 1u), q2 = q >> (2 * o.ltt);
+  const unsigned zo = q2 & ((1u << o.lzo) - 1u), tile = q2 >> o.lzo;
+  *x = (int)(sx * o.st + ((tile >> o.ltpr) << o.ltt) + (in >> o.ltt));
+  *y = (int)(sy * o.st + ((tile & ((1u << o.ltpr) - 1u)) << o.ltt) + (in & (unsigned)(o.tt - 1)));
+  *z = (int)(sz * o.zt + ((zo << o.lzi) | zin));
+  return *x < p.X && *y < p.Y && *z < p.Z;
+}
+
+__device__ __forceinline__ int64_t remap_block(unsigned b, int chunk_blocks, const SlabOrder& o) {
+  if (chunk_blocks <= 0) return b;
+  if (o.p2) {
+    const unsigned k = b >> 3;
+    return (((b & 7u) + 8u * (k >> o.lcb)) << o.lcb) | (k & ((1u << o.lcb) - 1u));
+  }
+  const int64_t grp = b & 7, k = b >> 3;
+  return (grp + 8 * (k / chunk_blocks)) * chunk_blocks + k % chunk_blocks;
+}
+
 __device__ __forceinline__ bool lattice_decode(const DenseParams& p, const SlabOrder& o, int64_t lb, int tid, int* x, int* y, int* z) {
   const int cb = o.st * o.st / 8;
   const int64_t sv = lb / cb;
@@ -129,10 +167,11 @@
 }
 
 typedef float dense_f4 __attribute__((ext_vector_type(4)));
-
-template <int ELEM> struct DenseElem { typedef float type; typedef float4 load_t; static constexpr int Q = 1; };
-template <> struct DenseElem<CNRMA_ELEM_F16> { typedef uint16_t type; typedef uint4 load_t; static constexpr int Q = 2; };
-template <> struct DenseElem<CNRMA_ELEM_BF16> { typedef uint16_t type; typedef uint4 load_t; static constexpr int Q = 2; };
+typedef unsigned int dense_u4 __attribute__((ext_vector_type(4)));
+
+template <int ELEM> struct DenseElem { typedef float type; typedef float4 load_t; typedef dense_f4 vec_t; static constexpr int Q = 1; };
+template <> struct DenseElem<CNRMA_ELEM_F16> { typedef uint16_t type; typedef uint4 load_t; typedef dense_u4 vec_t; static constexpr int Q = 2; };
+template <> struct DenseElem<CNRMA_ELEM_BF16> { typedef uint16_t type; typedef uint4 load_t; typedef dense_u4 vec_t; static constexpr int Q = 2; };
 
 __device__ __forceinline__ void store_run(float* o, float a, float b, float c, float d, int policy) {
   dense_f4 v = {a, b, c, d};
@@ -141,33 +180,43 @@
   else *reinterpret_cast<dense_f4*>(o) = v;
 }
 
+__device__ __forceinline__ bool block_voxel(const DenseParams& p, const SlabOrder& ord, int64_t lb, int tid, float* wx, float* wy,
+                                            float* wz, int64_t* lin) {
+  *wx = 0.f; *wy = 0.f; *wz = 0.f; *lin = -1;
+  bool in_grid;
+  if (ord.on) {
+    int x = 0, y = 0, z = 0;
+    in_grid = ord.on == 2 ? lattice_decode(p, ord, lb, tid, &x, &y, &z) : block_decode(p, ord, lb, tid, &x, &y, &z);
+    if (in_grid) {
+      *lin = ((int64_t)x * p.Y + y) * p.Z + z;
+      *wx = (float)x * p.vs + p.ox; *wy = (float)y * p.vs + p.oy; *wz = (float)z * p.vs + p.oz;
+    }
+  } else {
+    const int64_t g = lb * 256 + tid;
+    in_grid = g < (int64_t)p.X * p.Y * p.Z;
+    if (in_grid) { voxel_world(p, g, wx, wy, wz); *lin = g; }
+  }
+  return in_grid;
+}
+
 template <int LPV, int PIPE, int EPI, int ELEM = 0>
 __device__ __forceinline__ void accum_block(const DenseParams& p, const typename DenseElem<ELEM>::type* __restrict__ feat,
                                             const float* __restrict__ proj, float* __restrict__ volume,
                                             int32_t* __restrict__ count, int64_t lb, int c0, bool write_count,
-                                            const SlabOrder& ord, float* __restrict__ lds_wave, int tid) {
+                                            const SlabOrder& ord, float* __restrict__ lds_wave, int tid,
+                                            const unsigned long long* __restrict__ vmask = nullptr,
+                                            unsigned long long* __restrict__ vmask_out = nullptr) {
   constexpr int VPG = 64 / LPV;
   constexpr int Q = DenseElem<ELEM>::Q, CPL = 4 * Q;
   typedef typename DenseElem<ELEM>::type feat_t;
   typedef typename DenseElem<ELEM>::load_t load_t;
+  typedef typename DenseElem<ELEM>::vec_t vec_t;
   static_assert(EPI != 1 || ELEM == 0, "the LDS-transposed epilogue exists for fp32 maps only");
   const int64_t G = (int64_t)p.X * p.Y * p.Z;
   const int lane = tid & 63;
-  const int64_t g = lb * 256 + tid;
-  float wx = 0.f, wy = 0.f, wz = 0.f;
-  bool in_grid;
-  int64_t lin = -1;
-  if (ord.on) {
-    int x = 0, y = 0, z = 0;
-    in_grid = ord.on == 2 ? lattice_decode(p, ord, lb, tid, &x, &y, &z) : slab_decode(p, ord, g, &x, &y, &z);
-    if (in_grid) {
-      lin = ((int64_t)x * p.Y + y) * p.Z + z;
-      wx = (float)x * p.vs + p.ox; wy = (float)y * p.vs + p.oy; wz = (float)z * p.vs + p.oz;
-    }
-  } else {
-    in_grid = g < G;
-    if (in_grid) { voxel_world(p, g, &wx, &wy, &wz); lin = g; }
-  }
+  float wx, wy, wz;
+  int64_t lin;
+  bool in_grid = block_voxel(p, ord, lb, tid, &wx, &wy, &wz, &lin);
   if (__ballot(in_grid) == 0ull) return;
   float4 acc[LPV * Q];
 #pragma unroll
@@ -184,12 +233,17 @@
   };
   auto gather = [&](int v, int pix, load_t* q) {
     const feat_t* fv = fbase + v * plane;
+    int pq[LPV];
+#pragma unroll
+    for (int grp = 0; grp < LPV; ++grp) pq[grp] = __shfl(pix, group_src_lane<LPV, EPI>(grp, vsel), 64);
 #pragma unroll
     for (int grp = 0; grp < LPV; ++grp) {
-      const int pq = __shfl(pix, group_src_lane<LPV, EPI>(grp, vsel), 64);
       if constexpr (ELEM == 0) q[grp] = make_float4(0.f, 0.f, 0.f, 0.f);
       else q[grp] = make_uint4(0u, 0u, 0u, 0u);
-      if (pq >= 0) q[grp] = *reinterpret_cast<const load_t*>(fv + (int64_t)pq * p.C);
+      if (pq[grp] >= 0) {
+        const vec_t t = *(const __attribute__((address_space(1))) vec_t*)(fv + (int64_t)pq[grp] * p.C);
+        q[grp].x = t.x; q[grp].y = t.y; q[grp].z = t.z; q[grp].w = t.w;
+      }
     }
   };
   auto add = [&](const load_t* q) {
@@ -207,15 +261,45 @@
   };
 
   if constexpr (PIPE == 1) {
-    int pix_n = pixel_of(0);
-    for (int v = 0; v < p.V; ++v) {
+    const int nw = (p.V + 63) >> 6;
+    const int64_t wave_words = (lb * 4 + __builtin_amdgcn_readfirstlane(tid >> 6)) * nw;
+    const unsigned long long* wm = vmask != nullptr ? vmask + wave_words : nullptr;
+    unsigned long long seen = 0ull;
+    auto word = [&](int w) -> unsigned long long {
+      if (wm != nullptr) return wm[w];
+      const int left = p.V - 64 * w;
+      return left >= 64 ? ~0ull : (1ull << left) - 1ull;
+    };
+    int w = 0;
+    unsigned long long m = word(0);
+    auto next_view = [&]() -> int {
+      while (m == 0ull) {
+        if (++w >= nw) return -1;
+        m = word(w);
+      }
+      const int v = 64 * w + __builtin_ctzll(m);
+      m &= m - 1ull;
+      return v;
+    };
+    int v = next_view();
+    int pix_n = v >= 0 ? pixel_of(v) : -1;
+    while (v >= 0) {
       const int pix = pix_n;
       const bool any = __ballot(pix >= 0) != 0ull;
       load_t q[LPV];
       if (any) gather(v, pix, q);
       cnt += pix >= 0 ? 1 : 0;
-      pix_n = (v + 1 < p.V) ? pixel_of(v + 1) : -1;
+      const int vn = next_view();
+      if (vmask_out != nullptr) {
+        if (any) seen |= 1ull << (v & 63);
+        if (vn < 0 || (vn >> 6) != (v >> 6)) {
+          if (lane == 0) vmask_out[wave_words + (v >> 6)] = seen;
+          seen = 0ull;
+        }
+      }
+      pix_n = vn >= 0 ? pixel_of(vn) : -1;
       if (any) add(q);
+      v = vn;
     }
   } else {
     load_t q0[LPV], q1[LPV];
@@ -245,7 +329,7 @@
     int x = 0, y = 0, z = 0;
     const int64_t g2 = lb * 256 + t2;
     bool in2;
-    if (ord.on) in2 = ord.on == 2 ? lattice_decode(p, ord, lb, t2, &x, &y, &z) : slab_decode(p, ord, g2, &x, &y, &z);
+    if (ord.on) in2 = ord.on == 2 ? lattice_decode(p, ord, lb, t2, &x, &y, &z) : block_decode(p, ord, lb, t2, &x, &y, &z);
     else { in2 = g2 < G; z = (int)(g2 % p.Z); y = (int)((g2 / p.Z) % p.Y); x = (int)(g2 / p.Z / p.Y); }
     in_grid = in2;
     lin = in2 ? ((int64_t)x * p.Y + y) * p.Z + z : -1;
@@ -344,7 +428,9 @@
                                                                      int32_t* __restrict__ count, int chunk_blocks,
                                                                      int64_t n_phys, SlabOrder ord,
                                                                      unsigned int* __restrict__ bar,
-                                                                     const float* const* __restrict__ feat_ref) {
+                                                                     const float* const* __restrict__ feat_ref,
+                                                                     const unsigned long long* __restrict__ vmask,
+                                                                     unsigned long long* __restrict__ vmask_out, int sweep0) {
   if (feat_ref != nullptr) feat = *feat_ref;
   __shared__ float lds[EPI == 1 ? 4 * (4 * LPV) * 65 : 1];
   float* lds_wave = lds + (EPI == 1 ? (threadIdx.x >> 6) * (4 * LPV) * 65 : 0);
@@ -363,15 +449,12 @@
       }
   } else {
     int64_t lb = blockIdx.x;
-    int sweep = blockIdx.y;
+    int sweep = blockIdx.y + sweep0;
     if (ord.own > 0) {
       sweep = (int)(lb & 7);
       lb >>= 3;
-    } else if (chunk_blocks > 0) {
-      const int64_t grp = lb & 7, k = lb >> 3;
-      lb = (grp + 8 * (k / chunk_blocks)) * chunk_blocks + k % chunk_blocks;
-    }
-    accum_block<LPV, PIPE, EPI>(p, feat, proj, volume, count, lb, sweep * (4 * LPV), sweep == 0, ord, lds_wave, (int)threadIdx.x);
+    } else lb = remap_block(blockIdx.x, chunk_blocks, ord);
+    accum_block<LPV, PIPE, EPI>(p, feat, proj, volume, count, lb, sweep * (4 * LPV), sweep == 0, ord, lds_wave, (int)threadIdx.x, vmask, vmask_out);
   }
 }
 
@@ -381,15 +464,13 @@
                                                                          float* __restrict__ volume,
                                                                          int32_t* __restrict__ count, int chunk_blocks,
                                                                          SlabOrder ord,
-                                                                         const uint16_t* const* __restrict__ feat_ref) {
+                                                                         const uint16_t* const* __restrict__ feat_ref,
+                                                                         const unsigned long long* __restrict__ vmask,
+                                                                         unsigned long long* __restrict__ vmask_out, int sweep0) {
   if (feat_ref != nullptr) feat = *feat_ref;
-  int64_t lb = blockIdx.x;
-  if (chunk_blocks > 0) {
-    const int64_t grp = lb & 7, k = lb >> 3;
-    lb = (grp + 8 * (k / chunk_blocks)) * chunk_blocks + k % chunk_blocks;
-  }
-  const int sweep = blockIdx.y;
-  accum_block<LPV, 1, 0, ELEM>(p, feat, proj, volume, count, lb, sweep * (8 * LPV), sweep == 0, ord, nullptr, (int)threadIdx.x);
+  const int64_t lb = remap_block(blockIdx.x, chunk_blocks, ord);
+  const int sweep = blockIdx.y + sweep0;
+  accum_block<LPV, 1, 0, ELEM>(p, feat, proj, volume, count, lb, sweep * (8 * LPV), sweep == 0, ord, nullptr, (int)threadIdx.x, vmask, vmask_out);
 }
 
 #ifdef CNRMA_EXPERIMENTS
@@ -422,9 +503,25 @@
 #define CNRMA_DENSE_TUNE k_dense_tune
 #endif
 
+static void slab_shifts(SlabOrder& o, int64_t gx, int64_t cb) {
+  auto lg = [](int v) { int l = 0; while (l < 30 && (1 << l) < v) ++l; return (1 << l) == v ? l : -1; };
+  const int lst = lg(o.st), lzt = lg(o.zt), ltt = lg(o.tt), lzi = lg(o.zi);
+  if (lst < 0 || lzt < 0 || ltt < 0 || lzi < 0 || 2 * lst + lzt < 8 || gx >= ((int64_t)1 << 31) ||
+      cb != ((int64_t)1 << (2 * lst + lzt - 8))) return;
+  o.p2 = 1; o.lcb = 2 * lst + lzt - 8; o.lzi = lzi; o.ltt = ltt; o.lzo = lzt - lzi; o.ltpr = lst - ltt;
+}
+
+static unsigned long long* view_mask_table(const DenseParams& p, void* workspace, int64_t workspace_bytes, int64_t gx) {
+  const int64_t room = CNRMA_DENSE_MASK_BYTES(p.X, p.Y, p.Z, p.V);
+  if (workspace == nullptr || (reinterpret_cast<uintptr_t>(workspace) & 7) != 0 || workspace_bytes < CNRMA_DENSE_WORKSPACE_BYTES + room) return nullptr;
+  if (gx * 4 * ((p.V + 63) / 64) * 8 > room) return nullptr;
+  return reinterpret_cast<unsigned long long*>(static_cast<char*>(workspace) + CNRMA_DENSE_WORKSPACE_BYTES);
+}
+
 template <int LPV>
 int launch_accum_coop(const DenseParams& p, const float* feat, const float* proj, float* volume, int32_t* count,
-                      unsigned int* bar, hipStream_t st, const float* const* feat_ref = nullptr) {
+                      void* workspace, int64_t workspace_bytes, hipStream_t st, const float* const* feat_ref = nullptr) {
+  unsigned int* bar = (workspace != nullptr && workspace_bytes >= CNRMA_DENSE_WORKSPACE_BYTES) ? static_cast<unsigned int*>(workspace) : nullptr;
   const DenseTune t = CNRMA_DENSE_TUNE;
   if (feat_ref != nullptr && t.variant != 1) return CNRMA_EINVAL;
   const int64_t G = (int64_t)p.X * p.Y * p.Z;
@@ -443,6 +540,7 @@
   int64_t gx = nb;
   if (cb > 0 && (nb >= 16 * cb || ord.on)) gx = ceil_div(ceil_div(nb, cb), 8) * 8 * cb;
   else cb = 0;
+  if (ord.on) slab_shifts(ord, gx, cb);
 #ifdef CNRMA_EXPERIMENTS
   if (t.variant == 0) {
     int64_t launch_x = gx;
@@ -471,26 +569,31 @@
   const int n_sweeps = (int)ceil_div(p.C, 4 * LPV);
   if (t.own && !lock && ord.on && n_sweeps == 8 && nb * 8 < ((int64_t)1 << 31)) ord.own = 1;
   dim3 grid(lock ? (unsigned)(ord.groups * cb) : (ord.own ? (unsigned)(nb * 8) : (unsigned)gx), (lock || ord.own) ? 1u : (unsigned)n_sweeps);
+  unsigned long long* vmask = (!lock && !ord.own && t.pipe != 2 && n_sweeps > 1) ? view_mask_table(p, workspace, workspace_bytes, gx) : nullptr;
+  auto launch = [&](dim3 grid, int sweep0, const unsigned long long* vin, unsigned long long* vout) -> int {
 #ifdef CNRMA_EXPERIMENTS
 #define CNRMA_DENSE_LAUNCH(PIPE, EPI)                                                                                      \
   do {                                                                                                                     \
     if (lock)                                                                                                              \
       hipLaunchKernelGGL((backproject_accum_pipe_kernel<LPV, PIPE, EPI, 1>), grid, dim3(256), 0, st, p, feat, proj, volume, \
-                         count, (int)cb, gx, ord, bar, feat_ref);                                                          \
+                         count, (int)cb, gx, ord, bar, feat_ref, vin, vout, sweep0);                                       \
     else                                                                                                                   \
       hipLaunchKernelGGL((backproject_accum_pipe_kernel<LPV, PIPE, EPI, 0>), grid, dim3(256), (size_t)t.ldspad * 1024, st, p,  \
-                         feat, proj, volume, count, (int)cb, gx, ord, bar, feat_ref);                                     \
+                         feat, proj, volume, count, (int)cb, gx, ord, bar, feat_ref, vin, vout, sweep0);                  \
   } while (0)
   if (t.pipe == 2) { if (t.epi) CNRMA_DENSE_LAUNCH(2, 1); else if (t.zrun) CNRMA_DENSE_LAUNCH(2, 0); else CNRMA_DENSE_LAUNCH(2, 2); }
   else             { if (t.epi) CNRMA_DENSE_LAUNCH(1, 1); else if (t.zrun) CNRMA_DENSE_LAUNCH(1, 0); else CNRMA_DENSE_LAUNCH(1, 2); }
 #undef CNRMA_DENSE_LAUNCH
 #else
-  (void)lock;
   hipLaunchKernelGGL((backproject_accum_pipe_kernel<LPV, 1, 0, 0>), grid, dim3(256), 0, st, p, feat, proj, volume, count, (int)cb, gx,
-                     ord, bar, feat_ref);
+                     ord, bar, feat_ref, vin, vout, sweep0);
 #endif
-  CNRMA_LAUNCH_CHECK();
-  return 0;
+    CNRMA_LAUNCH_CHECK();
+    return 0;
+  };
+  if (vmask == nullptr) return launch(grid, 0, nullptr, nullptr);
+  const int rc = launch(dim3(grid.x, 1u), 0, nullptr, vmask);
+  return rc != 0 ? rc : launch(dim3(grid.x, (unsigned)(n_sweeps - 1)), 1, vmask, nullptr);
 }
 
 __global__ __launch_bounds__(256) void backproject_index_kernel(DenseParams p, const float* __restrict__ proj,
@@ -537,16 +640,15 @@
   if (V <= 0 || C <= 0 || H <= 0 || W <= 0 || X <= 0 || Y <= 0 || Z <= 0) return CNRMA_EINVAL;
   DenseParams p{V, C, H, W, X, Y, Z, voxel_size, ox, oy, oz};
   hipStream_t st = as_stream(stream);
-  unsigned int* bar = (workspace != nullptr && workspace_bytes >= CNRMA_DENSE_WORKSPACE_BYTES) ? static_cast<unsigned int*>(workspace) : nullptr;
 #ifdef CNRMA_EXPERIMENTS
   const int l = CNRMA_DENSE_TUNE.lpv;
-  if (l == 16 && C % 64 == 0) return launch_accum_coop<16>(p, feat_nhwc, proj, volume, count, bar, st, feat_ref);
-  if (l == 4 && C % 16 == 0) return launch_accum_coop<4>(p, feat_nhwc, proj, volume, count, bar, st, feat_ref);
+  if (l == 16 && C % 64 == 0) return launch_accum_coop<16>(p, feat_nhwc, proj, volume, count, workspace, workspace_bytes, st, feat_ref);
+  if (l == 4 && C % 16 == 0) return launch_accum_coop<4>(p, feat_nhwc, proj, volume, count, workspace, workspace_bytes, st, feat_ref);
 #endif
-  if (C % 32 == 0) return launch_accum_coop<8>(p, feat_nhwc, proj, volume, count, bar, st, feat_ref);
-  if (C % 16 == 0) return launch_accum_coop<4>(p, feat_nhwc, proj, volume, count, bar, st, feat_ref);
-  if (C % 8 == 0) return launch_accum_coop<2>(p, feat_nhwc, proj, volume, count, bar, st, feat_ref);
-  if (C % 4 == 0) return launch_accum_coop<1>(p, feat_nhwc, proj, volume, count, bar, st, feat_ref);
+  if (C % 32 == 0) return launch_accum_coop<8>(p, feat_nhwc, proj, volume, count, workspace, workspace_bytes, st, feat_ref);
+  if (C % 16 == 0) return launch_accum_coop<4>(p, feat_nhwc, proj, volume, count, workspace, workspace_bytes, st, feat_ref);
+  if (C % 8 == 0) return launch_accum_coop<2>(p, feat_nhwc, proj, volume, count, workspace, workspace_bytes, st, feat_ref);
+  if (C % 4 == 0) return launch_accum_coop<1>(p, feat_nhwc, proj, volume, count, workspace, workspace_bytes, st, feat_ref);
   if (feat_ref != nullptr) return CNRMA_EINVAL;
   return launch_accum<1>(p, feat_nhwc, proj, volume, count, st);
 }
@@ -573,28 +675,34 @@
 
 template <int LPV, int OCC>
 static int launch_accum_h16(const DenseParams& p, const uint16_t* feat, const uint16_t* const* feat_ref, int elem, const float* proj,
-                            float* volume, int32_t* count, hipStream_t st) {
+                            float* volume, int32_t* count, void* workspace, int64_t workspace_bytes, hipStream_t st) {
   constexpr DenseTune t{};
   SlabOrder ord{1, (int)ceil_div(p.X, t.st), (int)ceil_div(p.Y, t.st), (int)ceil_div(p.Z, t.zt), t.zt, t.st, t.tt, t.zi, t.nt, 0, 0, 8};
   const int64_t cb = (int64_t)t.st * t.st * t.zt / 256;
   const int64_t nb = (int64_t)ord.nsx * ord.nsy * ord.nsz * cb;
   const int64_t gx = ceil_div(ceil_div(nb, cb), 8) * 8 * cb;
-  dim3 grid((unsigned)gx, (unsigned)ceil_div(p.C, 8 * LPV));
-  if (elem == CNRMA_ELEM_F16)
-    hipLaunchKernelGGL((backproject_accum_h16_kernel<LPV, CNRMA_ELEM_F16, OCC>), grid, dim3(256), 0, st, p, feat, proj, volume, count,
-                       (int)cb, ord, feat_ref);
-  else
-    hipLaunchKernelGGL((backproject_accum_h16_kernel<LPV, CNRMA_ELEM_BF16, OCC>), grid, dim3(256), 0, st, p, feat, proj, volume, count,
-                       (int)cb, ord, feat_ref);
-  CNRMA_LAUNCH_CHECK();
-  return 0;
+  slab_shifts(ord, gx, cb);
+  const int n_sweeps = (int)ceil_div(p.C, 8 * LPV);
+  unsigned long long* vmask = n_sweeps > 1 ? view_mask_table(p, workspace, workspace_bytes, gx) : nullptr;
+  auto launch = [&](dim3 grid, int sweep0, const unsigned long long* vin, unsigned long long* vout) -> int {
+    if (elem == CNRMA_ELEM_F16)
+      hipLaunchKernelGGL((backproject_accum_h16_kernel<LPV, CNRMA_ELEM_F16, OCC>), grid, dim3(256), 0, st, p, feat, proj, volume, count,
+                         (int)cb, ord, feat_ref, vin, vout, sweep0);
+    else
+      hipLaunchKernelGGL((backproject_accum_h16_kernel<LPV, CNRMA_ELEM_BF16, OCC>), grid, dim3(256), 0, st, p, feat, proj, volume, count,
+                         (int)cb, ord, feat_ref, vin, vout, sweep0);
+    CNRMA_LAUNCH_CHECK();
+    return 0;
+  };
+  if (vmask == nullptr) return launch(dim3((unsigned)gx, (unsigned)n_sweeps), 0, nullptr, nullptr);
+  const int rc = launch(dim3((unsigned)gx, 1u), 0, nullptr, vmask);
+  return rc != 0 ? rc : launch(dim3((unsigned)gx, (unsigned)(n_sweeps - 1)), 1, vmask, nullptr);
 }
 
 extern "C" int cnrma_backproject_accum_h16(const void* feat_nhwc, const void* const* feat_nhwc_ref, int elem, const float* proj,
                                            int V, int C, int H, int W, int X, int Y, int Z, float voxel_size, float ox, float oy,
                                            float oz, float* volume, int32_t* count, void* workspace, int64_t workspace_bytes,
                                            void* stream) {
-  (void)workspace; (void)workspace_bytes;
   if (!elem16_known(elem) || (feat_nhwc == nullptr) == (feat_nhwc_ref == nullptr) || (reinterpret_cast<uintptr_t>(feat_nhwc) & 15) != 0)
     return CNRMA_EINVAL;
   if (V <= 0 || C <= 0 || C % 8 != 0 || H <= 0 || W <= 0 || X <= 0 || Y <= 0 || Z <= 0) return CNRMA_EINVAL;
@@ -607,11 +715,11 @@
 #ifdef CNRMA_EXPERIMENTS
   if (CNRMA_DENSE_TUNE.lpv == 8 || CNRMA_DENSE_TUNE.lpv == 4) lanes64 = CNRMA_DENSE_TUNE.lpv;
 #endif
-  if (C % 64 == 0 && lanes64 == 8) return launch_accum_h16<8, 3>(p, f, fr, elem, proj, volume, count, st);
+  if (C % 64 == 0 && lanes64 == 8) return launch_accum_h16<8, 3>(p, f, fr, elem, proj, volume, count, workspace, workspace_bytes, st);
 #endif
-  if (C % 32 == 0) return launch_accum_h16<4, 4>(p, f, fr, elem, proj, volume, count, st);
-  if (C % 16 == 0) return launch_accum_h16<2, 4>(p, f, fr, elem, proj, volume, count, st);
-  return launch_accum_h16<1, 4>(p, f, fr, elem, proj, volume, count, st);
+  if (C % 32 == 0) return launch_accum_h16<4, 4>(p, f, fr, elem, proj, volume, count, workspace, workspace_bytes, st);
+  if (C % 16 == 0) return launch_accum_h16<2, 4>(p, f, fr, elem, proj, volume, count, workspace, workspace_bytes, st);
+  return launch_accum_h16<1, 4>(p, f, fr, elem, proj, volume, count, workspace, workspace_bytes, st);
 }
 
 template <int LPV>
diff --git a/cn-rma_amd/pipeline.py b/cn-rma_amd/pipeline.py
--- a/cn-rma_amd/pipeline.py
+++ b/cn-rma_amd/pipeline.py
@@ -403,6 +403,12 @@
                 if torch.is_tensor(t) and t.is_cuda:
                     t.record_stream(self.stream)
 
+    def _dense_workspace(self):
+        if getattr(self, "_dense_ws", None) is None:
+            self._dense_ws = rma.dense_workspace(self.device, self.cfg.dims, self.shape_nhwc[0], self.shape_nhwc[3],
+                                                 self.feature_dtype in rma.ELEM_CODES)
+        return self._dense_ws
+
     def _trace(self):
         cfg, plan = self.cfg, self.plan
         plan.begin_static()
@@ -420,7 +426,8 @@
                     out["volume"], out["count"] = rma.backproject_accum(None, None, cfg.dims, cfg.voxel_size, cfg.origin,
                                                                         cfg.stride, proj_scaled=self.proj_scaled,
                                                                         feat_ref=self.feat_ref, shape=self.shape_nhwc,
-                                                                        feat_dtype=self.feature_dtype)
+                                                                        feat_dtype=self.feature_dtype,
+                                                                        workspace=self._dense_workspace())
             fixed = cfg.sample_seed is not None
             coords, feats, n_sel, info = rma.aggregate_points_static(
                 self.nhwc, self.proj_inv, self.tsdf, cfg.dims, cfg.voxel_size, cfg.origin, cfg.n_steps, cfg.thr,
@@ -612,7 +619,8 @@
             for b, h in enumerate(self.holders):
                 if self.dense:
                     vols.append(rma.backproject_accum(None, None, cfg.dims, cfg.voxel_size, cfg.origin, cfg.stride,
-                                                      proj_scaled=h.proj_scaled, feat_ref=h.feat_ref, shape=h.shape_nhwc))
+                                                      proj_scaled=h.proj_scaled, feat_ref=h.feat_ref, shape=h.shape_nhwc,
+                                                      workspace=h._dense_workspace()))
                 coords, feats, n_sel, info = rma.aggregate_points_static(
                     h.nhwc, h.proj_inv, h.tsdf, cfg.dims, cfg.voxel_size, cfg.origin, cfg.n_steps, cfg.thr,
                     max_points=cfg.max_points, seed=(cfg.sample_seed if fixed else 0x5EED) + 7919 * b * (0 if fixed else 1),
diff --git a/cn-rma_amd/rma.py b/cn-rma_amd/rma.py
--- a/cn-rma_amd/rma.py
+++ b/cn-rma_amd/rma.py
@@ -55,7 +55,7 @@
 
 
 def backproject_accum(features_nhwc, projections, dims, voxel_size, origin, stride, proj_scaled=None, feat_ref=None, shape=None,
-                      feat_dtype=torch.float32):
+                      feat_dtype=torch.float32, workspace=None):
     _lib.require_gpu()
     X, Y, Z = dims
     if feat_ref is not None:
@@ -68,7 +68,8 @@
     volume = torch.empty((C, X, Y, Z), dtype=torch.float32, device=dev)
     count = torch.empty((X, Y, Z), dtype=torch.int32, device=dev)
     st = stream()
-    ws = _dense_workspace(dev, st)
+    h16 = feat_dtype in ELEM_CODES if feat_ref is not None else _h16_readable(features_nhwc)
+    ws = workspace if workspace is not None else _dense_workspace(dev, st, dense_workspace_bytes(dims, V, C, h16))
     tail = (ptr(proj), V, C, H, W, X, Y, Z, float(voxel_size), float(origin[0]), float(origin[1]), float(origin[2]), ptr(volume),
             ptr(count), ptr(ws), ws.numel() * 4, st)
     if feat_ref is not None:
@@ -89,13 +90,38 @@
 _DENSE_KEYS = ("variant", "slab", "st", "zt", "tt", "zi", "chunk", "persist", "lpv", "pipe", "epi", "lockstep", "lattice", "nt", "own", "stagger", "groups", "ldspad", "zrun")
 
 
-def _dense_workspace(dev, st):
-    key = (dev.index if dev.index is not None else torch.cuda.current_device(), st)
+DENSE_WORKSPACE_BYTES = 1024
+DENSE_MASK_MIN_SWEEPS = 3
+
+
+def dense_mask_bytes(dims, V):
+    X, Y, Z = dims
+    return (((X + 31) // 32) * ((Y + 31) // 32) * ((Z + 31) // 32) + 7) * 512 * ((V + 63) // 64) * 8
+
+
+def dense_sweeps(C, h16=False):
+    if h16:
+        return -(-C // (8 * (4 if C % 32 == 0 else 2 if C % 16 == 0 else 1)))
+    return -(-C // (4 * (8 if C % 32 == 0 else 4 if C % 16 == 0 else 2 if C % 8 == 0 else 1)))
+
+
+def dense_workspace_bytes(dims, V, C=None, h16=False):
+    masks = C is None or dense_sweeps(C, h16) >= DENSE_MASK_MIN_SWEEPS
+    return DENSE_WORKSPACE_BYTES + (dense_mask_bytes(dims, V) if masks else 0)
+
+
+def dense_workspace(dev, dims, V, C=None, h16=False):
+    return torch.zeros((dense_workspace_bytes(dims, V, C, h16) + 3) // 4, dtype=torch.int32, device=dev)
+
+
+def _dense_workspace(dev, st, nbytes=0):
+    nbytes = max(int(nbytes), DENSE_WORKSPACE_BYTES)
+    key = (dev.index if dev.index is not None else torch.cuda.current_device(), st, nbytes)
     ws = _DENSE_WS.get(key)
     if ws is None:
         if len(_DENSE_WS) >= 64:
             _DENSE_WS.pop(next(iter(_DENSE_WS)))
-        ws = torch.zeros(256, dtype=torch.int32, device=dev)
+        ws = torch.zeros((nbytes + 3) // 4, dtype=torch.int32, device=dev)
         _DENSE_WS[key] = ws
     return ws
 
diff --git a/include/cnrma.h b/include/cnrma.h
--- a/include/cnrma.h
+++ b/include/cnrma.h
@@ -20,6 +20,9 @@
 int cnrma_nchw_to_nhwc_f32(const float* feat_nchw, float* feat_nhwc, int V, int C, int H, int W, void* stream);
 
 #define CNRMA_DENSE_WORKSPACE_BYTES 1024
+#define CNRMA_DENSE_MASK_BYTES(X, Y, Z, V)                                                                              \
+  ((((((int64_t)(X) + 31) / 32) * (((int64_t)(Y) + 31) / 32) * (((int64_t)(Z) + 31) / 32) + 7) * 512) *               \
+   (((int64_t)(V) + 63) / 64) * 8)
 int cnrma_backproject_accum_f32(const float* feat_nhwc, const float* proj, int V, int C, int H, int W,
                                 int X, int Y, int Z, float voxel_size, float ox, float oy, float oz,
                                 float* volume, int32_t* count, void* workspace, int64_t workspace_bytes, void* stream);
```

Result: faster. 64.18 scenes/s (median of 6 runs) (+2.0%).
